# BarisYazici/deep-rl-grasping

Measured on NVIDIA H100. Metric: SAC grad-steps/sec (batch 256, 64x64 depth), higher is better.
Workload: dtype bf16x3 (fp32-faithful split, f32 accumulate)

## Files before the change

deep-rl-grasping_b200/_lib.py:

```python
from __future__ import annotations

import ctypes as C
import os

_HERE = os.path.dirname(os.path.abspath(__file__))
LIB_PATH = os.path.join(_HERE, "libb200grasp.so")

B2G_PREC_FP32_SIMT, B2G_PREC_BF16X3, B2G_PREC_BF16 = 0, 1, 2
B2G_EINVAL, B2G_ECUDA, B2G_ESTATE = -1, -2, -3

SYMBOLS = [
    "b2g_last_error", "b2g_version", "b2g_nccl_unique_id", "b2g_sac_create", "b2g_sac_destroy", "b2g_sac_dp_export", "b2g_sac_dp_connect", "b2g_debug_dp_stamps", "b2g_debug_compact_host", "b2g_sync",
    "b2g_sac_create2", "b2g_param_count", "b2g_param_info", "b2g_get_param", "b2g_set_param", "b2g_get_grad", "b2g_get_adam",
    "b2g_reset_optimizer", "b2g_replay_add", "b2g_replay_size", "b2g_replay_get", "b2g_replay_info", "b2g_get_last_batch", "b2g_set_norm_stats", "b2g_sac_step",
    "b2g_sac_step_async", "b2g_sac_step_explicit", "b2g_sac_step_host_pipelined", "b2g_sac_pipeline_flush", "b2g_sac_act", "b2g_launches_per_step", "b2g_last_step_ms",
    "b2g_profile_step", "b2g_sac_state_save", "b2g_sac_state_load",
    "b2g_sac_observe_act", "b2g_sac_observe_add", "b2g_obs_rms_set", "b2g_obs_rms_get", "b2g_upload_bytes",
    "b2g_bdq_create", "b2g_bdq_destroy", "b2g_bdq_param_count", "b2g_bdq_param_info", "b2g_bdq_get_param", "b2g_bdq_set_param",
    "b2g_bdq_get_grad", "b2g_bdq_replay_add", "b2g_bdq_replay_size", "b2g_bdq_set_norm_stats", "b2g_bdq_step",
    "b2g_bdq_step_explicit", "b2g_bdq_act", "b2g_bdq_set_per_beta", "b2g_bdq_get_last_per", "b2g_bdq_state_save", "b2g_bdq_state_load",
    "b2g_bdq_observe_act", "b2g_bdq_observe_add", "b2g_bdq_obs_rms_set", "b2g_bdq_obs_rms_get", "b2g_bdq_upload_bytes",
    "b2g_dqn_create", "b2g_dqn_destroy", "b2g_dqn_param_count", "b2g_dqn_param_info", "b2g_dqn_get_param", "b2g_dqn_set_param",
    "b2g_dqn_get_grad", "b2g_dqn_replay_add", "b2g_dqn_replay_size", "b2g_dqn_set_norm_stats", "b2g_dqn_step",
    "b2g_dqn_step_explicit", "b2g_dqn_set_per_beta", "b2g_dqn_get_last_per", "b2g_dqn_update_target", "b2g_dqn_act",
    "b2g_dqn_state_save", "b2g_dqn_state_load",
    "b2g_ppo_create", "b2g_ppo_destroy", "b2g_ppo_param_count", "b2g_ppo_param_info", "b2g_ppo_get_param", "b2g_ppo_set_param",
    "b2g_ppo_get_grad", "b2g_ppo_rollout_act", "b2g_ppo_rollout_reward", "b2g_ppo_rollout_reset", "b2g_ppo_rollout_get",
    "b2g_ppo_update", "b2g_ppo_train_step_explicit", "b2g_ppo_act", "b2g_ppo_get_step", "b2g_ppo_state_save", "b2g_ppo_state_load",
    "b2g_encoder_create", "b2g_encoder_destroy", "b2g_encoder_n_layers", "b2g_encoder_layer_shape", "b2g_encoder_set_weights",
    "b2g_encoder_encode", "b2g_debug_gemm", "b2g_debug_tensor_info", "b2g_debug_tensor",
    "b2g_autoencoder_create", "b2g_autoencoder_destroy", "b2g_autoencoder_n_layers", "b2g_autoencoder_layer_shape",
    "b2g_autoencoder_set_weights", "b2g_autoencoder_get_weights", "b2g_autoencoder_get_grad", "b2g_autoencoder_reset_optimizer",
    "b2g_autoencoder_set_dataset", "b2g_autoencoder_train_epoch", "b2g_autoencoder_evaluate", "b2g_autoencoder_predict",
    "b2g_autoencoder_step",
]

ENC_MAX_LAYERS = 8


class EncoderCfg(C.Structure):
    _fields_ = [
        ("height", C.c_int32), ("width", C.c_int32), ("channels", C.c_int32), ("n_layers", C.c_int32),
        ("filters", C.c_int32 * ENC_MAX_LAYERS), ("kernel", C.c_int32 * ENC_MAX_LAYERS), ("strides", C.c_int32 * ENC_MAX_LAYERS),
        ("encoding_dim", C.c_int32), ("alpha", C.c_float), ("max_batch", C.c_int32), ("device", C.c_int32),
    ]


class BdqCfg(C.Structure):
    _fields_ = [
        ("obs_dim", C.c_int32), ("n_branches", C.c_int32), ("n_bins", C.c_int32), ("trunk0", C.c_int32), ("trunk1", C.c_int32),
        ("branch_hidden", C.c_int32), ("batch", C.c_int32), ("buffer_capacity", C.c_int64), ("gamma", C.c_float),
        ("target_update_freq", C.c_int32), ("trunk_grad_rescale", C.c_int32), ("seed", C.c_uint64), ("device", C.c_int32),
        ("rank", C.c_int32), ("nranks", C.c_int32), ("nccl_id", C.c_void_p), ("nccl_lib", C.c_char_p),
        ("prioritized_replay", C.c_int32), ("per_alpha", C.c_float), ("per_eps", C.c_float),
    ]


class BdqMetrics(C.Structure):
    _fields_ = [("loss", C.c_float), ("mean_q", C.c_float), ("grad_norm", C.c_float), ("n_updates", C.c_int64)]

    def as_dict(self):
        return {n: getattr(self, n) for n, _ in self._fields_}


class DqnCfg(C.Structure):
    _fields_ = [
        ("obs_dim", C.c_int32), ("n_actions", C.c_int32), ("hidden0", C.c_int32), ("hidden1", C.c_int32), ("batch", C.c_int32),
        ("buffer_capacity", C.c_int64), ("gamma", C.c_float), ("seed", C.c_uint64), ("device", C.c_int32),
        ("prioritized_replay", C.c_int32), ("per_alpha", C.c_float), ("per_eps", C.c_float),
    ]


class DqnMetrics(C.Structure):
    _fields_ = [("loss", C.c_float), ("mean_q", C.c_float), ("mean_abs_td", C.c_float), ("grad_norm", C.c_float),
                ("n_clipped", C.c_int32), ("n_updates", C.c_int64)]

    def as_dict(self):
        return {n: getattr(self, n) for n, _ in self._fields_}


class PpoCfg(C.Structure):
    _fields_ = [
        ("obs_dim", C.c_int32), ("n_actions", C.c_int32), ("hidden0", C.c_int32), ("hidden1", C.c_int32), ("n_envs", C.c_int32),
        ("n_steps", C.c_int32), ("nminibatches", C.c_int32), ("noptepochs", C.c_int32), ("gamma", C.c_float), ("lam", C.c_float),
        ("ent_coef", C.c_float), ("vf_coef", C.c_float), ("max_grad_norm", C.c_float), ("seed", C.c_uint64), ("device", C.c_int32),
    ]


class PpoMetrics(C.Structure):
    _fields_ = [("policy_loss", C.c_float), ("value_loss", C.c_float), ("entropy", C.c_float), ("approxkl", C.c_float),
                ("clipfrac", C.c_float), ("grad_norm", C.c_float), ("n_updates", C.c_int64)]

    def as_dict(self):
        return {n: getattr(self, n) for n, _ in self._fields_}


class SacCfg(C.Structure):
    _fields_ = [
        ("obs_h", C.c_int32), ("obs_w", C.c_int32), ("obs_c", C.c_int32), ("obs_dim", C.c_int32),
        ("n_act", C.c_int32), ("hidden", C.c_int32), ("batch", C.c_int32), ("buffer_capacity", C.c_int64),
        ("gamma", C.c_float), ("tau", C.c_float), ("target_entropy", C.c_float), ("seed", C.c_uint64),
        ("precision", C.c_int32), ("device", C.c_int32), ("rank", C.c_int32), ("nranks", C.c_int32),
        ("nccl_id", C.c_void_p), ("nccl_lib", C.c_char_p),
    ]


class ReplayCfg(C.Structure):
    _fields_ = [("frame_capacity", C.c_int64), ("u8_plane_mask", C.c_uint32)]


class SacMetrics(C.Structure):
    _fields_ = [(n, C.c_float) for n in (
        "policy_loss", "qf1_loss", "qf2_loss", "value_loss", "ent_coef_loss", "entropy", "ent_coef",
        "grad_norm_pi", "grad_norm_values", "grad_ent", "mean_q1", "mean_q2", "mean_v", "mean_logp")] + \
        [("n_updates", C.c_int64)]

    def as_dict(self):
        return {n: getattr(self, n) for n, _ in self._fields_}


class B2GError(RuntimeError):
    def __init__(self, msg, code=None):
        super().__init__(msg)
        self.code = code


_lib = None


def load():
    global _lib
    if _lib is not None:
        return _lib
    if not os.path.exists(LIB_PATH):
        raise B2GError(f"{LIB_PATH} is missing: run ./build.sh (there is no CPU fallback for the learner path)")
    lib = C.CDLL(LIB_PATH)
    fp, dp, vp = C.POINTER(C.c_float), C.POINTER(C.c_double), C.c_void_p
    lib.b2g_last_error.restype = C.c_char_p
    lib.b2g_nccl_unique_id.argtypes = [vp, C.c_char_p]
    lib.b2g_sac_create.argtypes = [C.POINTER(SacCfg), C.POINTER(vp)]
    lib.b2g_sac_create2.argtypes = [C.POINTER(SacCfg), C.POINTER(ReplayCfg), C.POINTER(vp)]
    i64p = C.POINTER(C.c_int64)
    lib.b2g_replay_info.argtypes = [vp, i64p, i64p, i64p, i64p, i64p, i64p]
    lib.b2g_sac_destroy.argtypes = [vp]
    lib.b2g_sac_dp_export.argtypes = [vp, vp]
    lib.b2g_sac_dp_connect.argtypes = [vp, vp, C.c_int]
    lib.b2g_debug_dp_stamps.argtypes = [vp, C.POINTER(C.c_longlong)]
    lib.b2g_debug_compact_host.argtypes = [vp, vp, C.c_int, C.c_int, C.c_int, C.c_int]
    lib.b2g_sync.argtypes = [vp]
    lib.b2g_param_count.argtypes = [vp]
    lib.b2g_param_info.argtypes = [vp, C.c_int, C.POINTER(C.c_char_p), C.POINTER(C.c_int64), C.POINTER(C.c_int32),
                                   C.POINTER(C.c_int64)]
    for f in ("b2g_get_param", "b2g_set_param", "b2g_get_grad"):
        getattr(lib, f).argtypes = [vp, C.c_char_p, fp, C.c_size_t]
    lib.b2g_get_adam.argtypes = [vp, C.c_char_p, fp, fp, C.c_size_t]
    lib.b2g_reset_optimizer.argtypes = [vp]
    lib.b2g_replay_add.argtypes = [vp, fp, fp, fp, fp, fp, C.c_int64]
    lib.b2g_replay_size.argtypes = [vp]
    lib.b2g_replay_size.restype = C.c_int64
    lib.b2g_replay_get.argtypes = [vp, C.c_int64, fp, fp, fp, fp, fp]
    lib.b2g_get_last_batch.argtypes = [vp, C.POINTER(C.c_int32), fp, fp, fp]
    lib.b2g_set_norm_stats.argtypes = [vp, dp, dp, C.c_double, C.c_double, C.c_double, C.c_double, C.c_int, C.c_int]
    lib.b2g_sac_step.argtypes = [vp, C.c_int, C.c_float, C.POINTER(SacMetrics)]
    lib.b2g_sac_step_async.argtypes = [vp, C.c_int, C.c_float]
    lib.b2g_sac_step_explicit.argtypes = [vp, fp, fp, fp, fp, fp, fp, C.c_float, C.c_int, C.POINTER(SacMetrics), fp, fp]
    lib.b2g_sac_step_host_pipelined.argtypes = [vp, fp, fp, fp, fp, fp, fp, C.c_float, C.POINTER(SacMetrics), C.POINTER(C.c_int)]
    lib.b2g_sac_pipeline_flush.argtypes = [vp, C.POINTER(SacMetrics)]
    lib.b2g_sac_act.argtypes = [vp, fp, C.c_int, C.c_int, fp]
    lib.b2g_sac_observe_act.argtypes = [vp, fp, C.c_int, C.c_int, C.c_int, fp]
    lib.b2g_sac_observe_add.argtypes = [vp, fp, fp, fp, fp, fp, C.c_int, C.c_int]
    lib.b2g_obs_rms_set.argtypes = [vp, dp, dp, C.c_double]
    lib.b2g_obs_rms_get.argtypes = [vp, dp, dp, dp]
    lib.b2g_upload_bytes.argtypes = [vp, i64p, i64p]
    lib.b2g_launches_per_step.argtypes = [vp]
    lib.b2g_last_step_ms.argtypes = [vp]
    lib.b2g_last_step_ms.restype = C.c_float
    lib.b2g_profile_step.argtypes = [vp, C.c_float, C.POINTER(C.c_char_p), fp, C.c_int]
    for f in ("b2g_sac_state_save", "b2g_sac_state_load", "b2g_bdq_state_save", "b2g_bdq_state_load", "b2g_dqn_state_save",
              "b2g_dqn_state_load", "b2g_ppo_state_save", "b2g_ppo_state_load"):
        getattr(lib, f).argtypes = [vp, C.c_char_p]
    lib.b2g_bdq_create.argtypes = [C.POINTER(BdqCfg), C.POINTER(vp)]
    lib.b2g_bdq_destroy.argtypes = [vp]
    lib.b2g_bdq_param_count.argtypes = [vp]
    lib.b2g_bdq_param_info.argtypes = [vp, C.c_int, C.c_char_p, C.c_size_t, C.POINTER(C.c_int64), C.POINTER(C.c_int64), C.POINTER(C.c_int32)]
    for f in ("b2g_bdq_get_param", "b2g_bdq_set_param", "b2g_bdq_get_grad"):
        getattr(lib, f).argtypes = [vp, C.c_char_p, fp, C.c_size_t]
    lib.b2g_bdq_replay_add.argtypes = [vp, fp, fp, fp, fp, fp, C.c_int64]
    lib.b2g_bdq_replay_size.argtypes = [vp]
    lib.b2g_bdq_replay_size.restype = C.c_int64
    lib.b2g_bdq_set_norm_stats.argtypes = [vp, dp, dp, C.c_double, C.c_double, C.c_double, C.c_double, C.c_int, C.c_int]
    lib.b2g_bdq_step.argtypes = [vp, C.c_int, C.c_float, C.POINTER(BdqMetrics)]
    lib.b2g_bdq_step_explicit.argtypes = [vp, fp, fp, fp, fp, fp, fp, C.c_float, C.c_int, C.POINTER(BdqMetrics), fp]
    lib.b2g_bdq_act.argtypes = [vp, fp, C.c_int, C.POINTER(C.c_int32)]
    lib.b2g_bdq_set_per_beta.argtypes = [vp, C.c_float]
    lib.b2g_bdq_get_last_per.argtypes = [vp, C.POINTER(C.c_int32), fp, fp]
    lib.b2g_bdq_observe_act.argtypes = [vp, fp, C.c_int, C.c_int, C.c_float, C.POINTER(C.c_int32)]
    lib.b2g_bdq_observe_add.argtypes = [vp, fp, fp, fp, fp, fp, C.c_int, C.c_int]
    lib.b2g_bdq_obs_rms_set.argtypes = [vp, dp, dp, C.c_double]
    lib.b2g_bdq_obs_rms_get.argtypes = [vp, dp, dp, dp]
    lib.b2g_bdq_upload_bytes.argtypes = [vp, i64p, i64p]
    lib.b2g_dqn_create.argtypes = [C.POINTER(DqnCfg), C.POINTER(vp)]
    lib.b2g_dqn_destroy.argtypes = [vp]
    lib.b2g_dqn_param_count.argtypes = [vp]
    lib.b2g_dqn_param_info.argtypes = [vp, C.c_int, C.c_char_p, C.c_size_t, C.POINTER(C.c_int64), C.POINTER(C.c_int64), C.POINTER(C.c_int32)]
    for f in ("b2g_dqn_get_param", "b2g_dqn_set_param", "b2g_dqn_get_grad"):
        getattr(lib, f).argtypes = [vp, C.c_char_p, fp, C.c_size_t]
    lib.b2g_dqn_replay_add.argtypes = [vp, fp, fp, fp, fp, fp, C.c_int64]
    lib.b2g_dqn_replay_size.argtypes = [vp]
    lib.b2g_dqn_replay_size.restype = C.c_int64
    lib.b2g_dqn_set_norm_stats.argtypes = [vp, dp, dp, C.c_double, C.c_double, C.c_double, C.c_double, C.c_int, C.c_int]
    lib.b2g_dqn_step.argtypes = [vp, C.c_int, C.c_float, C.POINTER(DqnMetrics)]
    lib.b2g_dqn_step_explicit.argtypes = [vp, fp, fp, fp, fp, fp, fp, C.c_float, C.c_int, C.POINTER(DqnMetrics), fp]
    lib.b2g_dqn_set_per_beta.argtypes = [vp, C.c_float]
    lib.b2g_dqn_get_last_per.argtypes = [vp, C.POINTER(C.c_int32), fp, fp]
    lib.b2g_dqn_update_target.argtypes = [vp]
    lib.b2g_dqn_act.argtypes = [vp, fp, C.c_int, C.POINTER(C.c_int32), fp]
    lib.b2g_ppo_create.argtypes = [C.POINTER(PpoCfg), C.POINTER(vp)]
    lib.b2g_ppo_destroy.argtypes = [vp]
    lib.b2g_ppo_param_count.argtypes = [vp]
    lib.b2g_ppo_param_info.argtypes = [vp, C.c_int, C.c_char_p, C.c_size_t, C.POINTER(C.c_int64), C.POINTER(C.c_int64), C.POINTER(C.c_int32)]
    for f in ("b2g_ppo_get_param", "b2g_ppo_set_param", "b2g_ppo_get_grad"):
        getattr(lib, f).argtypes = [vp, C.c_char_p, fp, C.c_size_t]
    lib.b2g_ppo_rollout_act.argtypes = [vp, fp, fp]
    lib.b2g_ppo_rollout_reward.argtypes = [vp, fp, fp]
    lib.b2g_ppo_rollout_reset.argtypes = [vp]
    lib.b2g_ppo_rollout_get.argtypes = [vp, fp, fp, fp, fp, fp]
    lib.b2g_ppo_update.argtypes = [vp, fp, C.POINTER(C.c_int32), C.c_float, C.c_float, C.c_float, C.POINTER(PpoMetrics)]
    lib.b2g_ppo_train_step_explicit.argtypes = [vp, fp, fp, fp, fp, fp, C.c_float, C.c_float, C.c_float, C.c_int, C.POINTER(PpoMetrics)]
    lib.b2g_ppo_act.argtypes = [vp, fp, C.c_int, C.c_int, fp, fp, fp]
    lib.b2g_ppo_get_step.argtypes = [vp, i64p, i64p, C.POINTER(C.c_int32)]
    lib.b2g_encoder_create.argtypes = [C.POINTER(EncoderCfg), C.POINTER(vp)]
    lib.b2g_encoder_destroy.argtypes = [vp]
    lib.b2g_encoder_n_layers.argtypes = [vp]
    lib.b2g_encoder_layer_shape.argtypes = [vp, C.c_int, C.POINTER(C.c_int64), C.POINTER(C.c_int64)]
    lib.b2g_encoder_set_weights.argtypes = [vp, C.c_int, fp, C.c_size_t, fp, C.c_size_t]
    lib.b2g_encoder_encode.argtypes = [vp, fp, C.c_int, fp]
    lib.b2g_autoencoder_create.argtypes = [C.POINTER(EncoderCfg), C.POINTER(vp)]
    lib.b2g_autoencoder_destroy.argtypes = [vp]
    lib.b2g_autoencoder_n_layers.argtypes = [vp]
    lib.b2g_autoencoder_layer_shape.argtypes = [vp, C.c_int, C.POINTER(C.c_int64), C.POINTER(C.c_int64)]
    for f in ("b2g_autoencoder_set_weights", "b2g_autoencoder_get_weights", "b2g_autoencoder_get_grad"):
        getattr(lib, f).argtypes = [vp, C.c_int, fp, C.c_size_t, fp, C.c_size_t]
    lib.b2g_autoencoder_reset_optimizer.argtypes = [vp]
    lib.b2g_autoencoder_set_dataset.argtypes = [vp, fp, fp, C.c_int64]
    lib.b2g_autoencoder_train_epoch.argtypes = [vp, C.POINTER(C.c_int32), C.c_int64, C.c_int, C.c_float, dp]
    lib.b2g_autoencoder_evaluate.argtypes = [vp, C.c_int64, C.c_int64, dp]
    lib.b2g_autoencoder_predict.argtypes = [vp, fp, C.c_int, fp]
    lib.b2g_autoencoder_step.argtypes = [vp, fp, fp, C.c_int, C.c_float, C.c_int, dp]
    lib.b2g_debug_gemm.argtypes = [C.c_int, C.c_int, C.c_int, fp, fp, fp, C.c_int, C.c_int]
    lib.b2g_debug_tensor_info.argtypes = [vp, C.c_char_p, i64p, C.POINTER(C.c_int32), C.POINTER(C.c_int32)]
    lib.b2g_debug_tensor.argtypes = [vp, C.c_char_p, C.c_int, vp, C.c_size_t]
    _lib = lib
    return lib


def check(rc: int):
    if rc < 0:
        raise B2GError(f"libb200grasp error {rc}: {load().b2g_last_error().decode(errors='replace')}", rc)
    return rc


def default_nccl_lib():
    try:
        import importlib.util
        spec = importlib.util.find_spec("nvidia.nccl")
        if spec and spec.submodule_search_locations:
            p = os.path.join(list(spec.submodule_search_locations)[0], "lib", "libnccl.so.2")
            if os.path.exists(p):
                return p
    except Exception:
        pass
    return None
```

deep-rl-grasping_b200/csrc/cg.cu:

```cuda
#include <cuda_bf16.h>

#include <cstdio>
#include <cstdlib>

#include "cg.cuh"
#include "common.cuh"
#include "wgmma.cuh"

namespace b2g {
namespace {

constexpr int NMMA_WARPS = 8, NEPI_WARPS = CG_EPI_WARPS, NPROD_WARPS = 2;
constexpr int EPI_WARP0 = NMMA_WARPS, PROD_WARP0 = NMMA_WARPS + NEPI_WARPS;
static_assert(NEPI_WARPS == 4, "the epilogue is one warpgroup: one row of the 128-row tile per lane");
constexpr int NTHREADS = 32 * (PROD_WARP0 + 4);
constexpr int MMA_REGS = 168, EPI_REGS = 152, PROD_REGS = 24;
static_assert(2 * MMA_REGS + EPI_REGS + PROD_REGS <= 512, "register file");
constexpr int STG_BYTES = 2 * 64 * 16 * 4;

__device__ __forceinline__ uint32_t smem_u32(const void* p) { return (uint32_t)__cvta_generic_to_shared(p); }
__device__ __forceinline__ void mbar_init(uint32_t bar, uint32_t count) {
  asm volatile("mbarrier.init.shared::cta.b64 [%0], %1;" ::"r"(bar), "r"(count));
}
__device__ __forceinline__ void mbar_arrive(uint32_t bar) { asm volatile("mbarrier.arrive.shared::cta.b64 _, [%0];" ::"r"(bar) : "memory"); }
__device__ __forceinline__ void mbar_expect_tx(uint32_t bar, uint32_t bytes) {
  asm volatile("mbarrier.arrive.expect_tx.shared::cta.b64 _, [%0], %1;" ::"r"(bar), "r"(bytes) : "memory");
}
__device__ __forceinline__ void mbar_wait(uint32_t bar, uint32_t parity) {
  asm volatile(
      "{\n\t"
      ".reg .pred p;\n\t"
      "CG_WAIT:\n\t"
      "mbarrier.try_wait.parity.shared::cta.b64 p, [%0], %1;\n\t"
      "@p bra CG_DONE;\n\t"
      "bra CG_WAIT;\n\t"
      "CG_DONE:\n\t"
      "}" ::"r"(bar), "r"(parity)
      : "memory");
}
__device__ __forceinline__ bool elect_one() {
  uint32_t pred;
  asm volatile(
      "{\n\t"
      ".reg .pred p;\n\t"
      "elect.sync _|p, 0xffffffff;\n\t"
      "selp.u32 %0, 1, 0, p;\n\t"
      "}"
      : "=r"(pred));
  return pred != 0;
}
__device__ __forceinline__ uint64_t desc_at(uint64_t bits, uint32_t saddr) { return bits | (uint64_t)((saddr & 0x3FFFFu) >> 4); }

__device__ __forceinline__ void tma_load(uint32_t dst, const CUtensorMap* map, uint32_t bar, int rank, const int (&c)[5]) {
  switch (rank) {
    case 2:
      asm volatile("cp.async.bulk.tensor.2d.shared::cluster.global.tile.mbarrier::complete_tx::bytes [%0], [%1, {%3, %4}], [%2];" ::"r"(dst), "l"(map),
                   "r"(bar), "r"(c[0]), "r"(c[1])
                   : "memory");
      break;
    case 3:
      asm volatile("cp.async.bulk.tensor.3d.shared::cluster.global.tile.mbarrier::complete_tx::bytes [%0], [%1, {%3, %4, %5}], [%2];" ::"r"(dst),
                   "l"(map), "r"(bar), "r"(c[0]), "r"(c[1]), "r"(c[2])
                   : "memory");
      break;
    case 4:
      asm volatile("cp.async.bulk.tensor.4d.shared::cluster.global.tile.mbarrier::complete_tx::bytes [%0], [%1, {%3, %4, %5, %6}], [%2];" ::"r"(dst),
                   "l"(map), "r"(bar), "r"(c[0]), "r"(c[1]), "r"(c[2]), "r"(c[3])
                   : "memory");
      break;
    default:
      asm volatile("cp.async.bulk.tensor.5d.shared::cluster.global.tile.mbarrier::complete_tx::bytes [%0], [%1, {%3, %4, %5, %6, %7}], [%2];" ::"r"(
                       dst),
                   "l"(map), "r"(bar), "r"(c[0]), "r"(c[1]), "r"(c[2]), "r"(c[3]), "r"(c[4])
                   : "memory");
      break;
  }
}

struct CgPack { CgProblem p[CG_MAX_PROBLEMS]; };
struct Tile { int p, tm, tn, c_begin, c_end; };
struct Walker {
  int p = -1, next_start = 0, tile_start = 0, tiles_n = 1, per = 1, splits = 1, chunks = 0, cps = 0;
  __device__ __forceinline__ bool advance(const CgProblem* __restrict__ probs, int nprob, int tile) {
    bool changed = false;
    while (p < 0 || (p + 1 < nprob && tile >= next_start)) {
      ++p;
      const CgProblem& P = probs[p];
      tile_start = P.tile_start; tiles_n = P.tiles_n; per = P.tiles_m * P.tiles_n; splits = P.splits; chunks = P.chunks;
      cps = (chunks + splits - 1) / splits;
      next_start = p + 1 < nprob ? probs[p + 1].tile_start : 0x7fffffff;
      changed = true;
    }
    return changed;
  }
  __device__ __forceinline__ Tile tile(int t_abs) const {
    int t = t_abs - tile_start, split = 0;
    if (splits > 1) { split = t / per; t -= split * per; }
    Tile ti;
    ti.p = p;
    ti.tm = tiles_n == 1 ? t : t / tiles_n;
    ti.tn = t - ti.tm * tiles_n;
    ti.c_begin = split * cps;
    ti.c_end = min(chunks, ti.c_begin + cps);
    return ti;
  }
};

__device__ __forceinline__ uint32_t pack_bf16x2(float lo, float hi) {
  uint32_t d;
  asm("cvt.rn.bf16x2.f32 %0, %1, %2;" : "=r"(d) : "f"(hi), "f"(lo));
  return d;
}

template <int NT, int NPROD, int TRANS, int KS, int NACC>
__device__ __forceinline__ void mma_chunk(float (&acc)[NACC], uint32_t sbase, uint32_t a_off, uint32_t b_off, uint32_t a_ks, uint32_t b_ks,
                                          uint32_t a_ks2, uint64_t a_desc, uint64_t b_desc, uint32_t a_ps, uint32_t b_ps, uint32_t m_off) {
  constexpr int NPL = NPROD >= 6 ? 3 : (NPROD >= 3 ? 2 : 1), G = NT / 2;
  static_assert(NACC == G * NPL, "one accumulator group of NT columns per product order");
#pragma unroll
  for (int k = 0; k < KS; ++k) {
    uint64_t da[NPL], db[NPL];
#pragma unroll
    for (int pl = 0; pl < NPL; ++pl) {
      const uint32_t pa = sbase + (uint32_t)pl * a_ps + a_off + (uint32_t)(k & 1) * a_ks + (uint32_t)(k >> 1) * a_ks2 + m_off;
      const uint32_t pb = sbase + (uint32_t)pl * b_ps + b_off + (uint32_t)k * b_ks;
      da[pl] = desc_at(a_desc, pa);
      db[pl] = desc_at(b_desc, pb);
    }
    Wgmma<NT, TRANS>::mma(acc, da[0], db[0]);
    if constexpr (NPL >= 2) Wgmma<NT, TRANS>::mma(acc + G, da[0], db[1]);
    if constexpr (NPL >= 3) Wgmma<NT, TRANS>::mma(acc + 2 * G, da[0], db[2]);
    if constexpr (NPL >= 2) Wgmma<NT, TRANS>::mma(acc + G, da[1], db[0]);
    if constexpr (NPL >= 3) {
      Wgmma<NT, TRANS>::mma(acc + 2 * G, da[1], db[1]);
      Wgmma<NT, TRANS>::mma(acc + 2 * G, da[2], db[0]);
    }
  }
}

__device__ __forceinline__ void mbar_arrive_if(uint32_t bar, bool pred) {
  asm volatile(
      "{\n\t"
      ".reg .pred p;\n\t"
      "setp.ne.u32 p, %1, 0;\n\t"
      "@p mbarrier.arrive.shared::cta.b64 _, [%0];\n\t"
      "}" ::"r"(bar), "r"((uint32_t)pred)
      : "memory");
}
__device__ __forceinline__ void stamp_if(long long* dst, bool pred) {
  asm volatile(
      "{\n\t"
      ".reg .pred p;\n\t"
      ".reg .u64 t;\n\t"
      "mov.u64 t, %%clock64;\n\t"
      "setp.ne.u32 p, %1, 0;\n\t"
      "@p st.global.u64 [%0], t;\n\t"
      "}" ::"l"(dst), "r"((uint32_t)pred)
      : "memory");
}

template <int NT, int NPROD, int TRANS, int KS, class Body>
__device__ __forceinline__ void consume_tile(const CgProblem& P, const Tile& ti, uint32_t ring, uint32_t stg, int slot_bytes, int nstages, uint32_t& s,
                                             uint32_t& ph, uint64_t* bar_full, uint64_t* bar_empty, bool nomma, long long* ctrace, uint32_t& gc,
                                             bool handoff, uint32_t acc_buf, uint32_t& nb, uint64_t* acc_full, uint64_t* acc_empty, Body&& body) {
  constexpr int NGRP = NPROD >= 6 ? 3 : (NPROD >= 3 ? 2 : 1);
  constexpr int NACC = NT / 2 * NGRP;
  const int tid = threadIdx.x, lane = tid & 31, warp = tid >> 5;
  const int wg = warp >> 2, wl = warp & 3, half = wl >> 1;
  float acc[NACC];
#pragma unroll
  for (int j = 0; j < NACC; ++j) acc[j] = 0.f;
  const uint32_t a_ps = (uint32_t)P.a_pstride, b_ps = (uint32_t)P.b_pstride, a_off = P.a_off, b_off = P.b_off, a_ks = P.a_kstep, b_ks = P.b_kstep;
  const uint32_t a_ks2 = P.a_kstep2;
  const uint64_t a_desc = P.a_desc, b_desc = P.b_desc;
  const uint32_t m_off = (uint32_t)wg * (uint32_t)P.a_moff;
  uint32_t prev = 0;
  if (nomma) {
    for (int c = ti.c_begin; c < ti.c_end; ++c, ++gc) {
      mbar_wait(smem_u32(&bar_full[s]), (ph >> s) & 1u);
      mbar_arrive_if(smem_u32(&bar_empty[s]), lane == 0);
      ph ^= 1u << s;
      if (++s == (uint32_t)nstages) s = 0;
    }
  } else {
    for (int c = ti.c_begin; c < ti.c_end; ++c, ++gc) {
      long long* const tr = ctrace + gc * 8;
      const bool stamp = ctrace != nullptr && lane == 0 && gc < 64;
      stamp_if(tr + 3, stamp);
      mbar_wait(smem_u32(&bar_full[s]), (ph >> s) & 1u);
      stamp_if(tr + 4, stamp);
      wg_arrive();
      mma_chunk<NT, NPROD, TRANS, KS>(acc, ring + s * (uint32_t)slot_bytes, a_off, b_off, a_ks, b_ks, a_ks2, a_desc, b_desc, a_ps, b_ps, m_off);
      wg_commit();
      wg_wait<1>();
      mbar_arrive_if(smem_u32(&bar_empty[prev]), lane == 0 && c > ti.c_begin);
      stamp_if(tr + 5, stamp);
      prev = s;
      ph ^= 1u << s;
      if (++s == (uint32_t)nstages) s = 0;
    }
    wg_wait<0>();
    mbar_arrive_if(smem_u32(&bar_empty[prev]), lane == 0);
  }
  if constexpr (NGRP > 2) {
#pragma unroll
    for (int j = 0; j < NT / 2; ++j) acc[j] = acc[j] + (acc[j + NT / 2] + acc[j + NT]);
  } else if constexpr (NGRP > 1) {
#pragma unroll
    for (int j = 0; j < NT / 2; ++j) acc[j] = acc[j] + acc[j + NT / 2];
  }
  if (handoff) {
    mbar_wait(smem_u32(acc_empty), (nb & 1u) ^ 1u);
    const uint32_t R = 64u * wg + 16u * wl + (uint32_t)(lane >> 2), sw = (uint32_t)(lane >> 2);
    const uint32_t rowa = acc_buf + R * (uint32_t)(NT * 4) + (uint32_t)((lane & 1) * 8);
#pragma unroll
    for (int j = 0; j < NT / 8; ++j)
#pragma unroll
      for (int h = 0; h < 2; ++h) {
        const uint32_t a = rowa + (uint32_t)h * (8u * NT * 4) + ((((uint32_t)(2 * j) + (uint32_t)((lane & 3) >> 1)) ^ sw) << 4);
        asm volatile("st.shared.v2.f32 [%0], {%1,%2};" ::"r"(a), "f"(acc[4 * j + 2 * h]), "f"(acc[4 * j + 2 * h + 1]) : "memory");
      }
    __syncwarp();
    mbar_arrive_if(smem_u32(acc_full), lane == 0);
    ++nb;
    return;
  }
  const int rrow = 32 * (wl & 1) + lane;
  const uint32_t wstg = stg + (uint32_t)wg * 4096u;
#pragma unroll
  for (int R = 0; R < (NT + 63) / 64; ++R) {
    float x[32];
#pragma unroll
    for (int t = 0; t < 4; ++t) {
      const int c0 = 64 * R + 16 * t;
      if (c0 < NT) {
        asm volatile("bar.sync %0, 128;" ::"r"(1 + wg) : "memory");
#pragma unroll
        for (int jj = 0; jj < 2; ++jj)
#pragma unroll
          for (int h = 0; h < 2; ++h) {
            const int row = 16 * wl + (lane >> 2) + 8 * h, chunk = 2 * jj + ((lane & 3) >> 1);
            const int j = c0 / 8 + jj;
            const uint32_t a = wstg + (uint32_t)row * 64u + (uint32_t)((chunk ^ ((row >> 1) & 3)) << 4) + (uint32_t)((lane & 1) * 8);
            asm volatile("st.shared.v2.f32 [%0], {%1,%2};" ::"r"(a), "f"(acc[4 * j + 2 * h]), "f"(acc[4 * j + 2 * h + 1]) : "memory");
          }
        asm volatile("bar.sync %0, 128;" ::"r"(1 + wg) : "memory");
        if (half == (t >> 1)) {
#pragma unroll
          for (int cc = 0; cc < 4; ++cc) {
            const uint32_t a = wstg + (uint32_t)rrow * 64u + (uint32_t)((cc ^ ((rrow >> 1) & 3)) << 4);
            float* xd = x + 16 * (t & 1) + 4 * cc;
            asm volatile("ld.shared.v4.f32 {%0,%1,%2,%3}, [%4];" : "=f"(xd[0]), "=f"(xd[1]), "=f"(xd[2]), "=f"(xd[3]) : "r"(a));
          }
        }
      }
    }
    const int g = 2 * R + half;
    if (32 * g < NT) body(g, x);
  }
}

struct RowOff {
  long long roff = 0, rmoff = 0;
  int ri0 = 0, ri1 = 0;
  bool ok = true;
  __device__ __forceinline__ void set(const CgProblem& Q, int r) {
    const int d0 = Q.d0, d1 = Q.d1;
    const int i0 = r % d0, i12 = r / d0, i1 = i12 % d1, i2 = i12 / d1;
    roff = Q.o_base + (long long)i0 * Q.o0 + (long long)i1 * Q.o1 + (long long)i2 * Q.o2;
    if (Q.rgrp_rows > 0) roff += Q.rgrp_off[min(r / Q.rgrp_rows, 7)];
    rmoff = Q.m_base + (long long)i0 * Q.m0 + (long long)i1 * Q.m1 + (long long)i2 * Q.m2;
    ri0 = i0; ri1 = i1;
    ok = Q.lim_i0 <= 0 || i0 < Q.lim_i0;
  }
};

__global__ void __launch_bounds__(NTHREADS, 1)
cg_kernel(const __grid_constant__ CgPack pk, int nprob, int total_tiles, const CUtensorMap* __restrict__ maps, int max_stages,
          int dbg, long long* __restrict__ trace) {
  const CgProblem* __restrict__ probs = pk.p;
  extern __shared__ uint8_t smem_raw[];
  __shared__ __align__(8) uint64_t bar_full[CG_MAX_STAGES], bar_empty[CG_MAX_STAGES], acc_full, acc_empty;
  const int tid = threadIdx.x, lane = tid & 31;
  const int warp = __shfl_sync(0xffffffffu, tid >> 5, 0);
  const int trace_cta = dbg >> 8;
  const bool dbg_noload = dbg & 1, dbg_nomma = dbg & 2, dbg_nostore = dbg & 4, dbg_nost = dbg & 16;
  if (tid == 0) {
    for (int s = 0; s < max_stages; ++s) { mbar_init(smem_u32(&bar_full[s]), 1); mbar_init(smem_u32(&bar_empty[s]), NMMA_WARPS); }
    mbar_init(smem_u32(&acc_full), NMMA_WARPS);
    mbar_init(smem_u32(&acc_empty), NEPI_WARPS);
    asm volatile("fence.mbarrier_init.release.cluster;" ::: "memory");
  }
  __syncthreads();
  const uint32_t stg = (smem_u32(smem_raw) + 1023u) & ~1023u;
  const uint32_t ring = stg + STG_BYTES;
  pdl_trigger();
  pdl_wait();

  if (warp >= PROD_WARP0) {
    asm volatile("setmaxnreg.dec.sync.aligned.u32 %0;" ::"n"(PROD_REGS));
    const int pw = warp - PROD_WARP0;
    if (pw >= NPROD_WARPS) return;
    {
      uint32_t gc = 0, s = 0, ph = 0, nbuf = 0;
      int slot_bytes = 0, nstages = 1;
      bool handoff = false;
      Walker w;
      int n2 = 1, nloads = 0, planes = 0, tx = 0;
      const int* tab = nullptr;
      for (int tile = blockIdx.x; tile < total_tiles; tile += gridDim.x) {
        if (w.advance(probs, nprob, tile)) {
          const CgProblem& P = probs[w.p];
          n2 = P.n2; nloads = P.nloads; planes = P.planes; tx = P.tx_bytes; tab = P.tm_tab; handoff = cg_epi_handoff(P.epi);
          if (P.slot_bytes != slot_bytes || P.nstages != nstages) {
            for (int q = 0; q < nstages; ++q) mbar_wait(smem_u32(&bar_empty[q]), ((ph >> q) & 1u) ^ 1u);
            if (nbuf) {
              mbar_wait(smem_u32(&acc_full), (nbuf - 1) & 1u);
              mbar_wait(smem_u32(&acc_empty), (nbuf - 1) & 1u);
              asm volatile("fence.proxy.async.shared::cta;" ::: "memory");
            }
            slot_bytes = P.slot_bytes; nstages = P.nstages; s = 0;
          }
        }
        const Tile ti = w.tile(tile);
        const CgProblem& P = probs[ti.p];
        if (handoff && ti.c_end > ti.c_begin) ++nbuf;
        if (P.dep_ctr) {
          const int* __restrict__ ctr = P.dep_ctr;
          const int x0 = P.dep_by_chunk ? ti.c_begin : ti.tm, x1 = P.dep_by_chunk ? ti.c_end : ti.tm + 1;
          const int lo = x0 * P.dep_rows / P.dep_rows_tile, hi = min(P.dep_tiles - 1, (x1 * P.dep_rows - 1) / P.dep_rows_tile);
          const int expect = P.dep_expect * NEPI_WARPS;
          for (int j = lo + lane; j <= hi; j += 32) {
            int seen;
            do {
              asm volatile("ld.acquire.gpu.global.s32 %0, [%1];" : "=r"(seen) : "l"(ctr + j) : "memory");
              if (seen < expect) __nanosleep(100);
            } while (seen < expect);
          }
          __syncwarp();
          asm volatile("fence.proxy.async.global;" ::: "memory");
        }
        int base[CG_MAX_LOADS][5];
#pragma unroll
        for (int l = 0; l < CG_MAX_LOADS; ++l) {
          if (l < nloads) {
            const CgLoad& L = P.ld[l];
#pragma unroll
            for (int d = 0; d < 5; ++d) base[l][d] = L.c0[d] + ti.tm * L.d_tm[d] + ti.tn * L.d_tn[d];
            if (tab) { base[l][1] += tab[(ti.tm * CG_MAX_LOADS + l) * 2]; base[l][2] += tab[(ti.tm * CG_MAX_LOADS + l) * 2 + 1]; }
          }
        }
        int c1 = n2 > 1 ? ti.c_begin / n2 : 0, c2 = ti.c_begin - c1 * n2;
        for (int c = ti.c_begin; c < ti.c_end; ++c, ++gc) {
          const bool tr = trace && blockIdx.x == trace_cta && pw == 0 && gc < 64 && lane == 0;
          if (tr) trace[gc * 8 + 0] = clock64();
          mbar_wait(smem_u32(&bar_empty[s]), ((ph >> s) & 1u) ^ 1u);
          if (tr) trace[gc * 8 + 1] = clock64();
          const uint32_t full = smem_u32(&bar_full[s]);
          const bool leader = elect_one();
          if (dbg_noload) { if (pw == 0 && leader) mbar_arrive(full); }
          else {
            if (pw == 0 && leader) mbar_expect_tx(full, (uint32_t)tx);
            const uint32_t sbase = ring + s * (uint32_t)slot_bytes;
            int j = 0;
#pragma unroll
            for (int l = 0; l < CG_MAX_LOADS; ++l) {
              if (l < nloads) {
                const CgLoad& L = P.ld[l];
                int crd[5];
#pragma unroll
                for (int d = 0; d < 5; ++d) crd[d] = base[l][d] + c1 * L.d_c1[d] + c2 * L.d_c2[d];
                if (L.plane_box) {
                  if ((j & (NPROD_WARPS - 1)) == pw && leader) tma_load(sbase + (uint32_t)L.smem_off, maps + L.map, full, L.rank, crd);
                  ++j;
                } else {
                  for (int pl = 0; pl < planes; ++pl, ++j) {
#pragma unroll
                    for (int d = 2; d < 5; ++d) if (d == L.rank - 1) crd[d] = pl;
                    if ((j & (NPROD_WARPS - 1)) == pw && leader)
                      tma_load(sbase + (uint32_t)(pl * L.plane_stride + L.smem_off), maps + L.map, full, L.rank, crd);
                  }
                }
              }
            }
          }
          if (tr) { trace[gc * 8 + 2] = clock64(); trace[gc * 8 + 6] = ti.p * 100000 + ti.tm * 10 + ti.tn; }
          if (++c2 == n2) { c2 = 0; ++c1; }
          ph ^= 1u << s;
          if (++s == (uint32_t)nstages) s = 0;
        }
      }
    }
  } else if (warp < NMMA_WARPS) {
    asm volatile("setmaxnreg.inc.sync.aligned.u32 %0;" ::"n"(MMA_REGS));
    const int q = 2 * (warp >> 2) + (warp & 1);
    uint32_t it = 0, s = 0, ph = 0, gc = 0, nb = 0;
    int slot_bytes = 0, nstages = 1;
    Walker w;
    long long* const ctrace = trace && blockIdx.x == trace_cta && warp == 0 ? trace : nullptr;
    const int r = q * 32 + lane;
    int epi = 0, rows_tile = 0, lim_rows = 0, umma_n = 0, n_valid = 0, shape = 0;
    bool handoff = false;
    uint32_t acc_buf = 0;
    long long o_tm = 0;
    RowOff ro;
    for (int tile = blockIdx.x; tile < total_tiles; tile += gridDim.x) {
      if (w.advance(probs, nprob, tile)) {
        const CgProblem& Q = probs[w.p];
        epi = Q.epi; rows_tile = Q.rows_tile; lim_rows = Q.lim_rows; umma_n = Q.umma_n; n_valid = Q.n_valid; o_tm = Q.o_tm;
        ro.set(Q, r);
        shape = cg_shape_key(Q.umma_n, Q.nprod, Q.mn_major != 0, Q.ksteps);
        if (Q.slot_bytes != slot_bytes || Q.nstages != nstages) { slot_bytes = Q.slot_bytes; nstages = Q.nstages; s = 0; }
        handoff = cg_epi_handoff(epi);
        acc_buf = ring + (uint32_t)(nstages * slot_bytes);
      }
      const Tile ti = w.tile(tile);
      if (ti.c_end <= ti.c_begin) continue;
      const CgProblem& P = probs[ti.p];
      const bool valid0 = r < rows_tile && ti.tm * rows_tile + r < lim_rows && ro.ok;
      const long long off0 = ro.roff + (long long)ti.tm * o_tm;
      const int n0 = ti.tn * umma_n;
      const bool tre = trace && blockIdx.x == trace_cta && warp == 0 && lane == 0 && it < 16;
      if (tre) trace[512 + it * 4 + 0] = clock64();
      auto body = [&](int g, float (&x)[32]) {
        const int ng = n0 + 32 * g;
        if (dbg_nostore || ng >= n_valid || !valid0) return;
        float* dst = P.out_f + off0 + (long long)(ng >> 5) * P.f_grp;
        if (epi == CG_EPI_RAW) {
          if (P.atomic) {
#pragma unroll
            for (int j = 0; j < 8; ++j)
              asm volatile("red.global.add.v4.f32 [%0], {%1,%2,%3,%4};" ::"l"(dst + 4 * j), "f"(x[4 * j]), "f"(x[4 * j + 1]), "f"(x[4 * j + 2]),
                           "f"(x[4 * j + 3])
                           : "memory");
          } else {
#pragma unroll
            for (int j = 0; j < 8; ++j) *reinterpret_cast<float4*>(dst + 4 * j) = make_float4(x[4 * j], x[4 * j + 1], x[4 * j + 2], x[4 * j + 3]);
          }
          return;
        }
        const float sc = P.scale;
        if (P.atomic) {
#pragma unroll
          for (int j = 0; j < 8; ++j)
            asm volatile("red.global.add.v4.f32 [%0], {%1,%2,%3,%4};" ::"l"(dst + 4 * j), "f"(x[4 * j] * sc), "f"(x[4 * j + 1] * sc),
                         "f"(x[4 * j + 2] * sc), "f"(x[4 * j + 3] * sc)
                         : "memory");
        } else {
#pragma unroll
          for (int j = 0; j < 8; ++j)
            *reinterpret_cast<float4*>(dst + 4 * j) = make_float4(x[4 * j] * sc, x[4 * j + 1] * sc, x[4 * j + 2] * sc, x[4 * j + 3] * sc);
          if (P.dp_n > 1) {
            const int i4 = (int)((dst - P.dp_gbase) >> 2), per4 = P.dp_per4;
#pragma unroll
            for (int j = 0; j < 8; ++j) {
              const int owner = (i4 + j) / per4;
              if (owner != P.dp_rank)
                reinterpret_cast<float4*>(P.dp_recv[owner])[(size_t)P.dp_rank * per4 + (i4 + j - owner * per4)] =
                    make_float4(x[4 * j] * sc, x[4 * j + 1] * sc, x[4 * j + 2] * sc, x[4 * j + 3] * sc);
            }
          }
        }
      };
#define CG_CONSUME(NT, NPROD, TRANS, KS)                                                                                                      \
  consume_tile<NT, NPROD, TRANS, KS>(P, ti, ring, stg, slot_bytes, nstages, s, ph, bar_full, bar_empty, dbg_nomma, ctrace, gc, handoff, acc_buf, \
                                     nb, &acc_full, &acc_empty, body)
      switch (shape) {
        case cg_shape_key(32, 6, false, 4): CG_CONSUME(32, 6, 0, 4); break;
        case cg_shape_key(64, 6, false, 4): CG_CONSUME(64, 6, 0, 4); break;
        case cg_shape_key(64, 3, false, 4): CG_CONSUME(64, 3, 0, 4); break;
        case cg_shape_key(128, 3, false, 4): CG_CONSUME(128, 3, 0, 4); break;
        case cg_shape_key(64, 3, true, 4): CG_CONSUME(64, 3, 1, 4); break;
        case cg_shape_key(64, 3, true, 9): CG_CONSUME(64, 3, 1, 9); break;
        case cg_shape_key(128, 3, true, 4): CG_CONSUME(128, 3, 1, 4); break;
        default: __trap();
      }
#undef CG_CONSUME
      if (tre) {
        trace[512 + it * 4 + 1] = clock64();
        trace[512 + it * 4 + 2] = handoff;
        trace[512 + it * 4 + 3] = ti.p * 100000 + ti.tm * 10 + ti.tn;
      }
      ++it;
    }
  } else {
    asm volatile("setmaxnreg.inc.sync.aligned.u32 %0;" ::"n"(EPI_REGS));
    const int ew = warp - EPI_WARP0;
    const int r = ew * 32 + lane;
    uint32_t ne = 0;
    int slot_bytes = 0, nstages = 1;
    Walker w;
    int epi = 0, rows_tile = 0, lim_rows = 0, umma_n = 0, out_planes = 0, grp_stride = 32, n_valid = 0, grp_tab = 0;
    bool handoff = false;
    uint32_t acc_buf = 0;
    long long o_tm = 0, m_tm = 0;
    RowOff ro;
    const float* __restrict__ bias = nullptr;
    const uint16_t* __restrict__ mask = nullptr;
    for (int tile = blockIdx.x; tile < total_tiles; tile += gridDim.x) {
      if (w.advance(probs, nprob, tile)) {
        const CgProblem& Q = probs[w.p];
        epi = Q.epi; rows_tile = Q.rows_tile; lim_rows = Q.lim_rows; umma_n = Q.umma_n; out_planes = Q.out_planes;
        grp_stride = Q.grp_stride; n_valid = Q.n_valid; o_tm = Q.o_tm; m_tm = Q.m_tm; bias = Q.bias; mask = Q.mask; grp_tab = Q.grp_tab;
        ro.set(Q, r);
        if (Q.slot_bytes != slot_bytes || Q.nstages != nstages) { slot_bytes = Q.slot_bytes; nstages = Q.nstages; }
        handoff = cg_epi_handoff(epi);
        acc_buf = ring + (uint32_t)(nstages * slot_bytes);
      }
      const Tile ti = w.tile(tile);
      if (ti.c_end <= ti.c_begin || !handoff) continue;
      const CgProblem& P = probs[ti.p];
      bool valid0 = r < rows_tile && ti.tm * rows_tile + r < lim_rows && ro.ok;
      long long off0 = ro.roff + (long long)ti.tm * o_tm;
      const long long moff0 = ro.rmoff + (long long)ti.tm * m_tm;
      if (P.tm_sub > 1) {
        const int tq = ti.tm / P.tm_sub, tr = ti.tm - tq * P.tm_sub;
        off0 = ro.roff + (long long)tq * o_tm + (long long)tr * P.o_sub;
        valid0 = valid0 && tr * P.d1 + ro.ri1 < P.lim_i1;
      }
      const int n0 = ti.tn * umma_n, ngroups = umma_n >> 5;
      auto group_at = [&](int g, bool& valid, long long& off, long long& moff) {
        const int ng = n0 + 32 * g;
        valid = valid0; off = off0; moff = moff0;
        if (grp_tab) {
          const int gg = ng >> 5;
          valid = valid0 && ro.ri0 < P.grp_lim0[gg] && ro.ri1 < P.grp_lim1[gg];
          off = off0 + P.grp_off[gg]; moff = moff0 + P.grp_moff[gg] - ng;
        }
      };
      const bool tre = trace && blockIdx.x == trace_cta && ew == 0 && lane == 0 && ne < 16;
      if (tre) trace[576 + ne * 4 + 0] = clock64();
      uint32_t mbits[4] = {0u, 0u, 0u, 0u};
      if (epi == CG_EPI_DGRAD && !dbg_nostore) {
#pragma unroll
        for (int g = 0; g < 4; ++g) {
          bool valid;
          long long off, moff;
          group_at(g, valid, off, moff);
          const int ng = n0 + 32 * g;
          if (g < ngroups && valid && ng < n_valid) {
            uint4 mk[4];
#pragma unroll
            for (int j = 0; j < 4; ++j) mk[j] = __ldg(reinterpret_cast<const uint4*>(mask + moff + ng) + j);
#pragma unroll
            for (int j = 0; j < 4; ++j) {
              const uint32_t wd[4] = {mk[j].x, mk[j].y, mk[j].z, mk[j].w};
#pragma unroll
              for (int uu = 0; uu < 4; ++uu) {
                if (wd[uu] & 0x00007FFFu) mbits[g] |= 1u << (8 * j + 2 * uu);
                if (wd[uu] & 0x7FFF0000u) mbits[g] |= 1u << (8 * j + 2 * uu + 1);
              }
            }
          }
        }
      }
      mbar_wait(smem_u32(&acc_full), ne & 1u);
      if (tre) trace[576 + ne * 4 + 1] = clock64();
      const bool split_fin = P.ws != nullptr;
      float* __restrict__ wsrow = split_fin ? P.ws + ((size_t)(ti.tm * w.tiles_n + ti.tn) * 128 + r) * umma_n : nullptr;
      auto body = [&](int g, float (&x)[32], int pass) {
        const int ng = n0 + 32 * g;
        bool valid;
        long long off, moff;
        group_at(g, valid, off, moff);
        if (pass == 0 && split_fin) {
#pragma unroll
          for (int j = 0; j < 8; ++j)
            asm volatile("red.global.add.v4.f32 [%0], {%1,%2,%3,%4};" ::"l"(wsrow + 32 * g + 4 * j), "f"(x[4 * j]), "f"(x[4 * j + 1]), "f"(x[4 * j + 2]),
                         "f"(x[4 * j + 3])
                         : "memory");
          return;
        }
        const bool live = !dbg_nostore && ng < n_valid;
        float4 bv[8];
        if (epi == CG_EPI_ACT && live) {
#pragma unroll
          for (int j = 0; j < 8; ++j) bv[j] = __ldg(reinterpret_cast<const float4*>(bias + (long long)(ng >> 5) * P.bias_grp) + j);
        }
        if (!live) return;
        if (epi == CG_EPI_ACT) {
#pragma unroll
          for (int j = 0; j < 8; ++j) {
            x[4 * j] = fmaxf(x[4 * j] + bv[j].x, 0.f); x[4 * j + 1] = fmaxf(x[4 * j + 1] + bv[j].y, 0.f);
            x[4 * j + 2] = fmaxf(x[4 * j + 2] + bv[j].z, 0.f); x[4 * j + 3] = fmaxf(x[4 * j + 3] + bv[j].w, 0.f);
          }
          if (P.f0 > 0 && valid && !dbg_nost) {
            float* dst = P.out_f + (long long)ti.tm * P.f_tm + (long long)r * P.f0 + (long long)(ng >> 5) * P.f_grp;
#pragma unroll
            for (int j = 0; j < 8; ++j) *reinterpret_cast<float4*>(dst + 4 * j) = make_float4(x[4 * j], x[4 * j + 1], x[4 * j + 2], x[4 * j + 3]);
          }
        } else {
          const uint32_t mb = g == 0 ? mbits[0] : g == 1 ? mbits[1] : g == 2 ? mbits[2] : mbits[3];
#pragma unroll
          for (int j = 0; j < 32; ++j)
            if (!((mb >> j) & 1u)) x[j] = 0.f;
          if (P.colsum) {
            float cs[32];
#pragma unroll
            for (int j = 0; j < 32; ++j) cs[j] = x[j];
#pragma unroll
            for (int wd = 16; wd >= 1; wd >>= 1) {
              const bool up = (lane & wd) != 0;
#pragma unroll
              for (int j = 0; j < wd; ++j) {
                const float send = up ? cs[j] : cs[j + wd], keep = up ? cs[j + wd] : cs[j];
                cs[j] = keep + __shfl_xor_sync(0xffffffffu, send, wd);
              }
            }
            atomicAdd(P.colsum + ((ng + lane) & P.colsum_mask), cs[0]);
          }
        }
        const long long gcol = grp_tab ? 0 : (long long)(ng >> 5) * grp_stride;
        const long long roff = off + gcol;
        const int q0 = lane & ~3, qi = lane & 3;
#pragma unroll 1
        for (int pl = 0; pl < out_planes; ++pl) {
          uint32_t pk[16];
#pragma unroll
          for (int j = 0; j < 16; ++j) {
            pk[j] = pack_bf16x2(x[2 * j], x[2 * j + 1]);
            x[2 * j] -= __uint_as_float(pk[j] << 16);
            x[2 * j + 1] -= __uint_as_float(pk[j] & 0xFFFF0000u);
          }
          if (dbg_nost) continue;
#pragma unroll
          for (int m = 1; m <= 2; m <<= 1) {
            const bool up = (lane & m) != 0;
#pragma unroll
            for (int c0 = 0; c0 < 4; ++c0) {
              if (c0 & m) continue;
              const int c1 = c0 | m;
#pragma unroll
              for (int u = 0; u < 4; ++u) {
                const uint32_t got = __shfl_xor_sync(0xffffffffu, up ? pk[4 * c0 + u] : pk[4 * c1 + u], m);
                if (up) pk[4 * c0 + u] = got; else pk[4 * c1 + u] = got;
              }
            }
          }
          uint16_t* const base = P.out_p[pl];
#pragma unroll
          for (int j = 0; j < 4; ++j) {
            const long long oj = __shfl_sync(0xffffffffu, roff, q0 + j);
            const bool vj = __shfl_sync(0xffffffffu, valid ? 1 : 0, q0 + j) != 0;
            if (vj) *reinterpret_cast<uint4*>(base + oj + 8 * qi) = make_uint4(pk[4 * j], pk[4 * j + 1], pk[4 * j + 2], pk[4 * j + 3]);
          }
        }
      };
      const uint32_t rowa = acc_buf + (uint32_t)(r * umma_n * 4), sw = (uint32_t)(r & 7);
      for (int g = 0; g < ngroups; ++g) {
        float x[32];
#pragma unroll
        for (int cc = 0; cc < 8; ++cc) {
          const uint32_t a = rowa + ((((uint32_t)(8 * g + cc)) ^ sw) << 4);
          asm volatile("ld.shared.v4.f32 {%0,%1,%2,%3}, [%4];" : "=f"(x[4 * cc]), "=f"(x[4 * cc + 1]), "=f"(x[4 * cc + 2]), "=f"(x[4 * cc + 3]) : "r"(a));
        }
        if (g == ngroups - 1) {
          __syncwarp();
          mbar_arrive_if(smem_u32(&acc_empty), lane == 0);
        }
        body(g, x, 0);
      }
      ++ne;
      bool last_arriver = !split_fin;
      if (split_fin) {
        __syncwarp();
        int old = 0;
        if (lane == 0) { __threadfence(); old = atomicAdd(P.ws_cnt + (ti.tm * w.tiles_n + ti.tn) * NEPI_WARPS + ew, 1); }
        old = __shfl_sync(0xffffffffu, old, 0);
        last_arriver = old == w.splits - 1;
        if (last_arriver) {
          __threadfence();
          if (lane == 0) P.ws_cnt[(ti.tm * w.tiles_n + ti.tn) * NEPI_WARPS + ew] = 0;
          for (int g = 0; g < ngroups; ++g) {
            float x[32];
#pragma unroll
            for (int j = 0; j < 8; ++j) {
              const float4 sum = __ldcg(reinterpret_cast<const float4*>(wsrow + 32 * g) + j);
              x[4 * j] = sum.x; x[4 * j + 1] = sum.y; x[4 * j + 2] = sum.z; x[4 * j + 3] = sum.w;
              __stcg(reinterpret_cast<float4*>(wsrow + 32 * g) + j, make_float4(0.f, 0.f, 0.f, 0.f));
            }
            body(g, x, 1);
          }
        }
      }
      __syncwarp();
      if (lane == 0 && P.done_ctr && last_arriver) {
        __threadfence();
        atomicAdd(P.done_ctr + ti.tm, 1);
      }
      if (tre) { trace[576 + (ne - 1) * 4 + 2] = clock64(); trace[576 + (ne - 1) * 4 + 3] = ti.p * 100000 + ti.tm * 10 + ti.tn; }
    }
  }
}

typedef CUresult (*EncodeTiledFn)(CUtensorMap*, CUtensorMapDataType, cuuint32_t, void*, const cuuint64_t*, const cuuint64_t*, const cuuint32_t*,
                                  const cuuint32_t*, CUtensorMapInterleave, CUtensorMapSwizzle, CUtensorMapL2promotion, CUtensorMapFloatOOBfill);
EncodeTiledFn g_encode = nullptr;

}

bool cg_shape_supported(int umma_n, int nprod, bool mn_major, int ksteps) {
  switch (cg_shape_key(umma_n, nprod, mn_major, ksteps)) {
    case cg_shape_key(32, 6, false, 4): case cg_shape_key(64, 6, false, 4): case cg_shape_key(64, 3, false, 4): case cg_shape_key(128, 3, false, 4):
    case cg_shape_key(64, 3, true, 4): case cg_shape_key(64, 3, true, 9): case cg_shape_key(128, 3, true, 4): return true;
    default: return false;
  }
}

int cg_smem_limit() { return 226 * 1024 - STG_BYTES; }

int cg_encode_map(CUtensorMap* out, const void* base, int rank, const uint64_t* dims, const uint64_t* strides_bytes, const uint32_t* box,
                  const uint32_t* elem_strides, int swizzle) {
  if (swizzle != 128 && swizzle != 64) return -1;
  if (!g_encode) {
    cudaDriverEntryPointQueryResult q;
    void* fn = nullptr;
    if (cudaGetDriverEntryPoint("cuTensorMapEncodeTiled", &fn, cudaEnableDefault, &q) != cudaSuccess || !fn || q != cudaDriverEntryPointSuccess) return -1;
    g_encode = (EncodeTiledFn)fn;
  }
  cuuint64_t gd[5], gs[5];
  cuuint32_t bx[5], es[5];
  for (int i = 0; i < rank; ++i) { gd[i] = dims[i]; bx[i] = box[i]; es[i] = elem_strides ? elem_strides[i] : 1; }
  for (int i = 0; i + 1 < rank; ++i) gs[i] = strides_bytes[i];
  const CUresult r = g_encode(out, CU_TENSOR_MAP_DATA_TYPE_BFLOAT16, (cuuint32_t)rank, const_cast<void*>(base), gd, gs, bx, es, CU_TENSOR_MAP_INTERLEAVE_NONE,
                              swizzle == 128 ? CU_TENSOR_MAP_SWIZZLE_128B : CU_TENSOR_MAP_SWIZZLE_64B, CU_TENSOR_MAP_L2_PROMOTION_L2_256B,
                              CU_TENSOR_MAP_FLOAT_OOB_FILL_NONE);
  return r == CUDA_SUCCESS ? 0 : (int)r;
}

unsigned long long cg_desc_bits(int swizzle, bool mn_major, int lbo) {
  const unsigned long long l = mn_major ? (unsigned)lbo : 16u, sbo = 8u * (unsigned)swizzle;
  return ((l >> 4) & 0x3FFF) << 16 | ((sbo >> 4) & 0x3FFF) << 32 | (unsigned long long)(swizzle == 128 ? 1 : 2) << 62;
}

int cg_finalize(CgGroup& g, int smem_budget) {
  int start = 0, slot = 0;
  g.flops = 0;
  for (int i = 0; i < g.n; ++i) {
    CgProblem& P = g.host[i];
    P.tile_start = start;
    start += P.tiles_m * P.tiles_n * P.splits;
    for (int l = 0; l < P.nloads; ++l) {
      CgLoad& L = P.ld[l];
      L.plane_stride = L.smem_off >= P.b_off ? P.b_pstride : P.a_pstride;
      if (L.plane_box && L.box_bytes != L.plane_stride) return -2;
    }
    const int need = P.b_off + P.planes * P.b_pstride;
    P.slot_bytes = (need + 1023) / 1024 * 1024;
    slot = slot > P.slot_bytes ? slot : P.slot_bytes;
  }
  g.total_tiles = start;
  const int avail = smem_budget - 1024 ;
  g.slot_bytes = slot; g.nstages = 0;
  int ring = 0;
  for (int i = 0; i < g.n; ++i) {
    CgProblem& P = g.host[i];
    const int acc = cg_epi_handoff(P.epi) ? cg_acc_bytes(P.umma_n) : 0;
    const int avail_ring = avail - acc;
    P.nstages = P.slot_bytes > 0 ? avail_ring / P.slot_bytes : 0;
    if (P.nstages > CG_MAX_STAGES) P.nstages = CG_MAX_STAGES;
    if (P.nstages < 2) return -1;
    P.slot_bytes = avail_ring / P.nstages / 1024 * 1024;
    g.nstages = g.nstages > P.nstages ? g.nstages : P.nstages;
    ring = ring > P.nstages * P.slot_bytes + acc ? ring : P.nstages * P.slot_bytes + acc;
  }
  g.ring_bytes = ring;
  return 0;
}

long long* g_cg_trace = nullptr;

cudaError_t cg_launch(const CgGroup& g, const CUtensorMap* dev_maps, int num_sms, cudaStream_t s, bool pdl, int debug_flags) {
  if (g.total_tiles <= 0 || (debug_flags & 8)) return cudaSuccess;
  static bool attr_set = false;
  if (!attr_set) {
    cudaError_t e = cudaFuncSetAttribute(cg_kernel, cudaFuncAttributeMaxDynamicSharedMemorySize, 226 * 1024);
    if (e != cudaSuccess) return e;
    attr_set = true;
  }
  const int smem = 1024 + STG_BYTES + g.ring_bytes;
  const int grid = g.total_tiles < num_sms ? g.total_tiles : num_sms;
  CgPack pk;
  static_assert(sizeof(CgPack) < 28 * 1024, "problem list must fit the kernel parameter space (32,764 B)");
  for (int i = 0; i < g.n; ++i) pk.p[i] = g.host[i];
  cudaError_t e = launch_pdl(cg_kernel, dim3(grid), dim3(NTHREADS), (size_t)smem, s, pdl, pk, g.n, g.total_tiles, dev_maps, g.nstages, debug_flags, g_cg_trace);
  if (e != cudaSuccess) fprintf(stderr, "cg_launch %s: %s (grid %d, %d threads, smem %d)\n", g.name, cudaGetErrorString(e), grid, NTHREADS, smem);
  return e;
}

}
```

deep-rl-grasping_b200/csrc/cg.cuh:

```cuda
#pragma once
#include <cuda.h>
#include <cuda_runtime.h>
#include <stdint.h>

namespace b2g {

constexpr int CG_MAX_LOADS = 4;
constexpr int CG_MAX_PROBLEMS = 16;
constexpr int CG_MAX_STAGES = 8;
constexpr int CG_MAX_PLANES = 3;
constexpr int CG_EPI_WARPS = 4;

enum CgEpiKind : int {
  CG_EPI_ACT = 0,
  CG_EPI_RAW = 1,
  CG_EPI_DGRAD = 2,
  CG_EPI_WGRAD = 3,
};
__host__ __device__ constexpr bool cg_epi_handoff(int epi) { return epi == CG_EPI_ACT || epi == CG_EPI_DGRAD; }
__host__ __device__ constexpr int cg_acc_bytes(int umma_n) { return 128 * umma_n * 4; }

struct CgLoad {
  int map;
  int rank;
  int box_bytes;
  int smem_off;
  int plane_stride;
  int plane_box;
  int c0[5];
  int d_tm[5], d_tn[5], d_c1[5], d_c2[5];
};

struct CgProblem {
  int tile_start, tiles_m, tiles_n, splits;
  int chunks, n2;
  int nloads, planes;
  int a_pstride, b_pstride;
  int tx_bytes;
  int slot_bytes, nstages;
  CgLoad ld[CG_MAX_LOADS];
  const int* tm_tab;
  int mn_major;
  unsigned long long a_desc, b_desc;
  int a_moff;
  int ksteps;
  int a_off, b_off;
  int a_kstep, b_kstep;
  int a_kstep2;
  int a_lbo, b_lbo;
  int umma_n;
  int nprod;
  int epi;
  int rows_tile;
  int lim_rows;
  int d0, d1;
  long long o_tm; int o0, o1, o2; long long o_base;
  int rgrp_rows;
  int rgrp_off[8];
  int lim_i0;
  int tm_sub;
  long long o_sub;
  int lim_i1;
  long long m_tm; int m0, m1, m2; long long m_base;
  int n_valid;
  int grp_stride;
  int grp_tab;
  int grp_off[8], grp_moff[8], grp_lim0[8], grp_lim1[8];
  int out_planes;
  uint16_t* out_p[CG_MAX_PLANES];
  float* out_f;
  long long f_tm; int f0;
  const float* bias;
  int bias_grp;
  long long f_grp;
  const uint16_t* mask;
  float* colsum;
  int colsum_mask;
  int atomic;
  float scale;
  int* done_ctr;
  const int* dep_ctr;
  int dep_rows, dep_rows_tile, dep_tiles, dep_expect;
  float* ws;
  int* ws_cnt;
  float* dp_recv[8];
  const float* dp_gbase;
  int dp_rank, dp_n, dp_per4;
  int dep_by_chunk;
};

struct CgGroup {
  CgProblem host[CG_MAX_PROBLEMS];
  int n = 0;
  int total_tiles = 0;
  int slot_bytes = 0, nstages = 0, ring_bytes = 0;
  const char* name = "";
  double flops = 0;
};

int cg_encode_map(CUtensorMap* out, const void* base, int rank, const uint64_t* dims, const uint64_t* strides_bytes, const uint32_t* box,
                  const uint32_t* elem_strides, int swizzle = 128);
unsigned long long cg_desc_bits(int swizzle, bool mn_major, int lbo);
int cg_finalize(CgGroup& g, int smem_budget);
cudaError_t cg_launch(const CgGroup& g, const CUtensorMap* dev_maps, int num_sms, cudaStream_t s, bool pdl, int debug_flags);
int cg_smem_limit();
__host__ __device__ constexpr int cg_shape_key(int umma_n, int nprod, bool mn_major, int ksteps) {
  return ksteps * 8192 + umma_n * 16 + nprod * 2 + (mn_major ? 1 : 0);
}
bool cg_shape_supported(int umma_n, int nprod, bool mn_major, int ksteps);

}
```

deep-rl-grasping_b200/csrc/engine_v2.cu:

```cuda
#include <cuda_bf16.h>

#include <algorithm>
#include <cstdio>
#include <cstdlib>
#include <cstring>

#include "sac_internal.cuh"

namespace b2g {
namespace {

struct Gather2Args {
  GatherArgs g;
  uint16_t* s1[2][3];
  uint16_t* fp[3][3];
  int KF;
};

__device__ __forceinline__ void split3(float y, uint16_t& p0, uint16_t& p1, uint16_t& p2) {
  const __nv_bfloat16 h0 = __float2bfloat16_rn(y);
  const float r1 = y - __bfloat162float(h0);
  const __nv_bfloat16 h1 = __float2bfloat16_rn(r1);
  const float r2 = r1 - __bfloat162float(h1);
  p0 = __bfloat16_as_ushort(h0); p1 = __bfloat16_as_ushort(h1); p2 = __bfloat16_as_ushort(__float2bfloat16_rn(r2));
}

template <int Ci>
__device__ __forceinline__ void s2d_half_block(const Gather2Args& a, const unsigned char* __restrict__ src, int it, int which, size_t b) {
  constexpr int CP = s2d_channels(Ci);
  const GatherArgs& g = a.g;
  const int npx = g.H * g.W * Ci;
  const int h = it & 1, X = (it >> 1) & 15, Y = it >> 5;
  const double clip_obs = g.normc[1];
  const bool norm_obs = g.normc[3] != 0.0;
  const float scale = g.scale;
#pragma unroll
  for (int rr = 0; rr < 2; ++rr) {
    const int e0 = ((4 * Y + 2 * h + rr) * g.W + 4 * X) * Ci;
    float y[4 * Ci];
#pragma unroll
    for (int q = 0; q < Ci; ++q) {
      const int e = e0 + 4 * q;
      const float4 v = frame_load4(src, g.fmt, npx, Ci, e);
      float t[4] = {v.x, v.y, v.z, v.w};
      if (norm_obs) {
        const double2 m0 = *reinterpret_cast<const double2*>(g.mean + e), m1 = *reinterpret_cast<const double2*>(g.mean + e + 2);
        const double2 i0 = *reinterpret_cast<const double2*>(g.var + e), i1 = *reinterpret_cast<const double2*>(g.var + e + 2);
        t[0] = (float)fmin(fmax(((double)t[0] - m0.x) * i0.x, -clip_obs), clip_obs);
        t[1] = (float)fmin(fmax(((double)t[1] - m0.y) * i0.y, -clip_obs), clip_obs);
        t[2] = (float)fmin(fmax(((double)t[2] - m1.x) * i1.x, -clip_obs), clip_obs);
        t[3] = (float)fmin(fmax(((double)t[3] - m1.y) * i1.y, -clip_obs), clip_obs);
      }
#pragma unroll
      for (int j = 0; j < 4; ++j) y[4 * q + j] = t[j];
    }
    uint32_t p[3][2 * CP];
#pragma unroll
    for (int k = 0; k < 4 * CP; k += 2) {
      uint16_t q[3][2];
#pragma unroll
      for (int u = 0; u < 2; ++u) {
        const int c = (k + u) / CP, ci = (k + u) % CP;
        if (ci < Ci) split3(y[c * Ci + ci] / scale, q[0][u], q[1][u], q[2][u]);
        else q[0][u] = q[1][u] = q[2][u] = 0;
      }
#pragma unroll
      for (int pl = 0; pl < 3; ++pl) p[pl][k / 2] = (uint32_t)q[pl][0] | ((uint32_t)q[pl][1] << 16);
    }
    const size_t o = b * 4096 * CP + (size_t)((Y * 16 + X) * 16 + 4 * (2 * h + rr)) * CP;
#pragma unroll
    for (int pl = 0; pl < 3; ++pl) {
      if constexpr (CP == 1) {
        *reinterpret_cast<uint2*>(a.s1[which][pl] + o) = make_uint2(p[pl][0], p[pl][1]);
      } else {
        uint4* d = reinterpret_cast<uint4*>(a.s1[which][pl] + o);
        d[0] = make_uint4(p[pl][0], p[pl][1], p[pl][2], p[pl][3]);
        d[1] = make_uint4(p[pl][4], p[pl][5], p[pl][6], p[pl][7]);
      }
    }
  }
}

template <int Ci>
__global__ void __launch_bounds__(512) gather2_kernel(Gather2Args a) {
  const GatherArgs& g = a.g;
  const int b = blockIdx.x, which = blockIdx.y, tid = threadIdx.x;
  const int HW = g.H * g.W, npx = HW * Ci;
  const int Ec = npx + 4;
  long long slot = b;
  if (g.indices) slot = g.indices[b];
  else if (g.rng_counters) {
    slot = philox_slot(g.seed, (unsigned long long)g.rng_counters[4], b, (unsigned long long)g.rng_counters[5]);
    if (g.ring_cap > 0) slot = ring_slot(g.rng_counters[6], (int)slot, g.ring_cap);
    if (g.indices_out && which == 0 && tid == 0) g.indices_out[b] = (int)slot;
  }
  const unsigned char* __restrict__ src =
      g.obs_frame ? g.frames + (size_t)(which ? g.next_frame : g.obs_frame)[slot] * g.frame_bytes
                  : reinterpret_cast<const unsigned char*>((which ? g.next_obs : g.obs) + (size_t)slot * Ec);
  const double clip_obs = g.normc[1];
  const bool norm_obs = g.normc[3] != 0.0;
  const float scale = g.scale;
  for (int it = tid; it < 512; it += blockDim.x) s2d_half_block<Ci>(a, src, it, which, b);
  if (tid == 0) {
    float yy = frame_elem(src, g.fmt, npx, Ci, npx);
    if (norm_obs) yy = (float)fmin(fmax(((double)yy - g.mean[npx]) * g.var[npx], -clip_obs), clip_obs);
    yy = yy / scale;
    uint16_t p0, p1, p2;
    split3(yy, p0, p1, p2);
    const size_t fo = (size_t)b * g.FS + g.feat_col, po = (size_t)b * a.KF + g.feat_col;
    if (which) { g.F_t[fo] = yy; a.fp[2][0][po] = p0; a.fp[2][1][po] = p1; a.fp[2][2][po] = p2; }
    else {
      g.F_pi[fo] = yy; g.F_v[fo] = yy;
      a.fp[0][0][po] = p0; a.fp[0][1][po] = p1; a.fp[0][2][po] = p2;
      a.fp[1][0][po] = p0; a.fp[1][1][po] = p1; a.fp[1][2][po] = p2;
    }
  }
  if (which == 0 && g.act) {
    const int feat_dim = g.feat_col + 1;
    if (tid < g.n_act) {
      const float av = g.act[slot * g.n_act + tid];
      g.F_v[(size_t)b * g.FS + feat_dim + tid] = av;
      uint16_t p0, p1, p2;
      split3(av, p0, p1, p2);
      const size_t po = (size_t)b * a.KF + feat_dim + tid;
      a.fp[1][0][po] = p0; a.fp[1][1][po] = p1; a.fp[1][2][po] = p2;
    }
    if (tid == 32) {
      float r = g.rew[slot];
      if (g.normc[4] != 0.0) r = (float)fmin(fmax((double)r * g.normc[0], -g.normc[2]), g.normc[2]);
      g.rew_out[b] = r;
      g.done_out[b] = g.done[slot];
    }
  }
}

struct Plane2Job {
  const float* src;
  uint16_t* dst[3];
  int R, N, np;
  int transpose;
  int ld, off0;
  int k1_ci;
  int tile_start;
};

constexpr int P2_SUB = 4;
__global__ void __launch_bounds__(256) planes2_kernel(const Plane2Job* __restrict__ jobs, const int* __restrict__ cta_job, int cta0) {
  __shared__ float tile[P2_SUB][64][33];
  const int cta = cta0 + blockIdx.x;
  const Plane2Job job = jobs[cta_job[cta]];
  const int t = cta - job.tile_start;
  const int strips_n = (job.N + 32 * P2_SUB - 1) / (32 * P2_SUB);
  const int r0 = (t / strips_n) * 64, nb = (t % strips_n) * 32 * P2_SUB;
  const int tid = threadIdx.x;
  const bool vec_ok = (job.N & 3) == 0;
  float4 v[P2_SUB][2];
#pragma unroll
  for (int q = 0; q < P2_SUB; ++q)
#pragma unroll
// ... 535 lines not shown
        CgProblem P = mnmajor(NB, 64, 2, 1, (B + 3) / 4);
        P.nloads = 3;
        for (int a = 0; a < 2; ++a) { P.ld[a] = mk_load(mA, 4, a * P.a_lbo); P.ld[a].d_c2[3] = 4; }
        P.ld[2] = mk_load(mB, 2, P.b_off); P.ld[2].d_c2[1] = 64;
        P.tm_tab = dtab;
        P.tiles_m = 5; P.tiles_n = 1;
        P.splits = std::max(1, std::min(P.chunks, std::max(14, (P.chunks + 15) / 16)));
        P.lim_rows = 576; P.o_tm = 128 * 64; P.o0 = 64; P.n_valid = 64;
        P.out_f = h->g(std::string(nets[n]) + "/cnn3/w"); P.atomic = 1;
        g.host[g.n++] = P;
      }
    }
    if (int rc = push_group(h, v.bwd_groups, g, "conv3_bwd")) return rc;
  }
  {
    CgGroup g;
    for (int n = 0; n < 2; ++n) {
      const int mA = add_maps(v, v.dZ2[n], NB, 4, {64, 6, 6, (uint64_t)B}, {128, 768, 4608}, {64, 8, 8, 2});
      const int mB = add_maps(v, v.W2n[n], NB, 2, {64, 512}, {128}, {64, 64}, {}, false);
      if (mA < 0 || mB < 0) return b2g_fail(B2G_ECUDA, "engine v2: cuTensorMapEncodeTiled failed (conv2 dgrad)");
      CgProblem P = kmajor(NB, 128, 4, 2, 128);
      P.tx_bytes = NB * (128 * 128 + 2 * 64 * 128);
      P.nloads = 3;
      P.ld[0] = mk_load(mA, 4, 0); P.ld[0].d_tm[3] = 2; P.ld[0].d_c1[2] = -1; P.ld[0].d_c2[1] = -1;
      for (int py = 0; py < 2; ++py) {
        P.ld[1 + py] = mk_load(mB, 2, P.b_off + py * 64 * 128);
        P.ld[1 + py].c0[1] = py * 128; P.ld[1 + py].d_c1[1] = 256; P.ld[1 + py].d_c2[1] = 64;
      }
      P.tiles_m = (B + 1) / 2;
      P.epi = CG_EPI_DGRAD; P.rows_tile = 128; P.lim_rows = B * 64;
      P.d0 = 8; P.d1 = 8;
      P.o_tm = 2 * 225 * 64; P.o0 = 2 * 64; P.o1 = 2 * 15 * 64; P.o2 = 225 * 64; P.o_base = n * 32;
      P.m_tm = 2 * 225 * 32; P.m0 = 2 * 32; P.m1 = 2 * 15 * 32; P.m2 = 225 * 32; P.m_base = 0;
      P.grp_tab = 1;
      for (int py = 0; py < 2; ++py)
        for (int px = 0; px < 2; ++px) {
          const int gg = py * 2 + px;
          P.grp_off[gg] = (py * 15 + px) * 64; P.grp_moff[gg] = (py * 15 + px) * 32;
          P.grp_lim0[gg] = (15 - px + 1) / 2; P.grp_lim1[gg] = (15 - py + 1) / 2;
        }
      P.n_valid = 128; P.out_planes = 2;
      for (int p = 0; p < 2; ++p) P.out_p[p] = v.dZ1[p];
      P.mask = v.H1[n][0];
      P.colsum = h->g(std::string(nets[n]) + "/cnn1/b"); P.colsum_mask = 31;
      g.host[g.n++] = P;
    }
    if (int rc = push_group(h, v.bwd_groups, g, "conv2_dgrad")) return rc;
  }
  {
    CgGroup g;
    for (int n = 0; n < 2; ++n) {
      const int mA = add_maps(v, v.H1[n], NB, 4, {64, 14, 15, (uint64_t)B}, {64, 15 * 64, 225 * 64}, {64, 12, 12, 4}, {1, 2, 2, 1});
      const int mB = add_maps(v, v.dZ2[n], NB, 2, {64, (uint64_t)B * 36}, {128}, {64, 144});
      if (mA < 0 || mB < 0) return b2g_fail(B2G_ECUDA, "engine v2: cuTensorMapEncodeTiled failed (conv2 wgrad)");
      CgProblem P = mnmajor(NB, 144, 2, 1, (B + 3) / 4);
      P.nloads = 3;
      for (int a = 0; a < 2; ++a) { P.ld[a] = mk_load(mA, 4, a * P.a_lbo); P.ld[a].c0[1] = 2 * a; P.ld[a].d_tm[2] = 1; P.ld[a].d_c2[3] = 4; }
      P.ld[2] = mk_load(mB, 2, P.b_off); P.ld[2].d_c2[1] = 144;
      P.tiles_m = 4; P.tiles_n = 1;
      P.splits = std::max(1, std::min(P.chunks, std::max(8, (P.chunks + 7) / 8)));
      P.lim_rows = 512; P.o_tm = 128 * 64; P.o0 = 64; P.n_valid = 64;
      P.out_f = h->g(std::string(nets[n]) + "/cnn2/w"); P.atomic = 1;
      g.host[g.n++] = P;
    }
    {
      const int mA = Cp == 1 ? add_maps(v, v.S[0], NB, 3, {32, 15, (uint64_t)B * 16}, {32, 512}, {32, 16, 4}, {}, true, 64)
                             : add_maps(v, v.S[0], NB, 3, {64, 16, (uint64_t)B * 16}, {128, 2048}, {64, 16, 4});
      const int mB = add_maps(v, v.dZ1, NB, 4, {64, 15, 15, (uint64_t)B}, {128, 15 * 128, 225 * 128}, {64, 16, 4, 1});
      if (mA < 0 || mB < 0) return b2g_fail(B2G_ECUDA, "engine v2: cuTensorMapEncodeTiled failed (conv1 wgrad)");
      CgProblem P = mnmajor(NB, 64, 2, 1, 4 * B);
      P.n2 = 4;
      if (Cp == 1) {
        P.a_pstride = 64 * 64; P.a_lbo = NB * P.a_pstride;
        P.b_off = 2 * P.a_lbo;
        P.tx_bytes = NB * (2 * 64 * 64 + 64 * 128);
        P.a_kstep = 16 * 64; P.a_kstep2 = 2 * P.a_kstep; P.a_desc = cg_desc_bits(64, true, P.a_lbo); P.a_moff = 0;
        P.nloads = 3;
        for (int a = 0; a < 2; ++a) { P.ld[a] = mk_load(mA, 3, a * P.a_lbo); P.ld[a].c0[2] = a; P.ld[a].d_c1[2] = 16; P.ld[a].d_c2[2] = 4; }
        P.tiles_m = 1;
        P.d0 = 4; P.d1 = 4; P.o0 = 32; P.o1 = 8 * 32;
        P.rgrp_rows = 16;
        for (int l = 0; l < 4; ++l) P.rgrp_off[l] = (32 * (l >> 1) + 4 * (l & 1)) * 32;
      } else {
        for (int l = 0; l < 2; ++l) {
          P.ld[l] = mk_load(mA, 3, l * P.a_lbo); P.ld[l].c0[1] = l; P.ld[l].d_tm[2] = 1; P.ld[l].d_c1[2] = 16; P.ld[l].d_c2[2] = 4;
        }
        P.nloads = 3;
        P.tiles_m = 2;
        P.d0 = 4; P.d1 = 4; P.o0 = 32; P.o1 = Ci * 32; P.o_tm = 32 * Ci * 32;
        P.lim_i0 = Ci;
        P.rgrp_rows = 16;
        for (int j = 0; j < 8; ++j) P.rgrp_off[j] = (8 * Ci * (j & 3) + 4 * Ci * (j >> 2)) * 32;
      }
      P.ld[P.nloads - 1] = mk_load(mB, 4, P.b_off); P.ld[P.nloads - 1].d_c1[3] = 1; P.ld[P.nloads - 1].d_c2[2] = 4;
      P.tiles_n = 1;
      P.splits = std::max(1, std::min(P.chunks, std::max(84 / P.tiles_m, (P.chunks + 15) / 16)));
      P.lim_rows = 64 * Cp; P.n_valid = 64;
      P.out_f = h->g("model/pi/cnn1/w"); P.f_grp = (long long)(h->g("model/values_fn/cnn1/w") - h->g("model/pi/cnn1/w")); P.atomic = 1;
      g.host[g.n++] = P;
    }
    if (int rc = push_group(h, v.bwd_groups, g, "conv_wgrad")) return rc;
  }
  int n_ctr = 0;
  {
    std::vector<const CgGroup*> parts;
    for (auto& g : v.fwd) parts.push_back(&g);
    std::vector<Wire> w;
    for (int n = 0; n < 3; ++n) {
      w.push_back({1, n, 0, n < 2 ? 0 : 1, 6, 1, 0});
      w.push_back({2, n, 1, n, 8 * 36, 108, 0});
      w.push_back({3, n, 2, n, 128 * 16, 128, 0});
      w.push_back({4, n, 3, n, 128, 128, 0});
    }
    if (int rc = fuse_groups(h, parts, w, "fwd_fused", v.fwd_fused, n_ctr)) return rc;
  }
  {
    std::vector<const CgGroup*> parts;
    for (auto& g : v.bwd_groups) parts.push_back(&g);
    std::vector<Wire> w;
    for (int n = 0; n < 2; ++n) {
      w.push_back({1, 2 * n, 0, n, 128, 128, 0});
      w.push_back({1, 2 * n + 1, 0, n, 64, 128, 1});
      w.push_back({2, 2 * n, 1, 2 * n, 3, 128, 0});
      w.push_back({2, 2 * n + 1, 1, 2 * n, 4, 128, 1});
      w.push_back({3, n, 2, 2 * n, 72, 108, 0});
      w.push_back({4, n, 2, 2 * n, 144, 108, 1});
    }
    w.push_back({4, 2, 3, 0, 1, 8, 1});
    w.push_back({4, 2, 3, 1, 1, 8, 1});
    if (int rc = fuse_groups(h, parts, w, "bwd_fused", v.bwd_fused, n_ctr)) return rc;
    std::vector<const CgGroup*> pa(parts.begin(), parts.begin() + 2), pb(parts.begin() + 2, parts.end());
    std::vector<Wire> wa, wb;
    for (int n = 0; n < 2; ++n) {
      wa.push_back({1, 2 * n, 0, n, 128, 128, 0});
      wa.push_back({1, 2 * n + 1, 0, n, 64, 128, 1});
      wb.push_back({1, n, 0, 2 * n, 72, 108, 0});
      wb.push_back({2, n, 0, 2 * n, 144, 108, 1});
    }
    wb.push_back({2, 2, 1, 0, 1, 8, 1});
    wb.push_back({2, 2, 1, 1, 1, 8, 1});
    if (int rc = fuse_groups(h, pa, wa, "bwd_fused_fc", v.bwd_fused, n_ctr)) return rc;
    if (int rc = fuse_groups(h, pb, wb, "bwd_fused_conv", v.bwd_fused, n_ctr)) return rc;
  }
  if (int rc = dev_alloc(h->allocs, h->stream, &v.dep_ctr, (size_t)n_ctr)) return rc;
  v.n_dep_ctr = n_ctr;
  bind_counters(v.fwd_fused, v.dep_ctr);
  bind_counters(v.bwd_fused, v.dep_ctr);
  if (int rc = dev_alloc(h->allocs, h->stream, &v.d_maps, v.maps.size())) return rc;
  CK(cudaMemcpyAsync(v.d_maps, v.maps.data(), v.maps.size() * sizeof(CUtensorMap), cudaMemcpyHostToDevice, h->stream));
  CK(cudaStreamSynchronize(h->stream));
  return 0;
}

int v2_planes(b2g_sac* h, bool backward, cudaStream_t s) {
  V2State& v = h->v2;
  const int cta0 = backward ? v.plane_ctas_fwd : 0, n = backward ? v.plane_ctas - v.plane_ctas_fwd : v.plane_ctas_fwd;
  planes2_kernel<<<n, 256, 0, s>>>((const Plane2Job*)v.plane_jobs, v.plane_cta_job, cta0);
  return 0;
}

int v2_gather(b2g_sac* h, const GatherArgs& ga, cudaStream_t s) {
  V2State& v = h->v2;
  Gather2Args a{};
  a.g = ga;
  for (int w = 0; w < 2; ++w)
    for (int p = 0; p < 3; ++p) a.s1[w][p] = v.S[w][p];
  for (int n = 0; n < 3; ++n) for (int p = 0; p < 3; ++p) a.fp[n][p] = v.F[n][p];
  a.KF = v.KF;
  const dim3 grid(ga.B, ga.next_obs || ga.next_frame ? 2 : 1);
  switch (h->Cimg) {
    case 1: gather2_kernel<1><<<grid, 512, 0, s>>>(a); break;
    case 2: gather2_kernel<2><<<grid, 512, 0, s>>>(a); break;
    case 3: gather2_kernel<3><<<grid, 512, 0, s>>>(a); break;
    default: gather2_kernel<4><<<grid, 512, 0, s>>>(a); break;
  }
  return 0;
}

extern long long* g_cg_trace;
static long long* s_trace_buf = nullptr;

int v2_launch(b2g_sac* h, const CgGroup& g, cudaStream_t s) {
  const char* tn = getenv("B2G_CG_TRACE");
  cudaStreamCaptureStatus cs0 = cudaStreamCaptureStatusNone;
  if (tn) cudaStreamIsCapturing(s, &cs0);
  if (tn && cs0 == cudaStreamCaptureStatusNone && std::string(tn) == g.name) {
    if (!s_trace_buf) cudaMalloc(&s_trace_buf, 640 * sizeof(long long));
    cudaMemsetAsync(s_trace_buf, 0, 640 * sizeof(long long), s);
    g_cg_trace = s_trace_buf;
    const char* tc = getenv("B2G_CG_TRACE_CTA");
    cudaError_t e = cg_launch(g, h->v2.d_maps, h->num_sms - h->v2.sm_reserve, s, false, h->v2.dbg | ((tc ? atoi(tc) : 0) << 8));
    g_cg_trace = nullptr;
    if (e != cudaSuccess) return b2g_fail(B2G_ECUDA, cudaGetErrorString(e));
    static int shots = 0;
    if (shots++ == 3) {
      long long t[640];
      cudaStreamSynchronize(s);
      cudaMemcpy(t, s_trace_buf, sizeof(t), cudaMemcpyDeviceToHost);
      const long long t0 = t[0];
      fprintf(stderr, "cg trace %s (cycles; per chunk: prod wait_start wait_done issued | mma wait_start full_seen committed)\n", g.name);
      for (int i = 0; i < 64 && t[i * 8 + 2]; ++i)
        fprintf(stderr, "  chunk %2d (p %lld tm %lld): %7lld %7lld %7lld | %7lld %7lld %7lld\n", i, t[i * 8 + 6] / 100000, t[i * 8 + 6] % 100000 / 10, t[i * 8] - t0,
                t[i * 8 + 1] - t0, t[i * 8 + 2] - t0, t[i * 8 + 3] - t0, t[i * 8 + 4] - t0, t[i * 8 + 5] - t0);
      for (int i = 0; i < 16 && t[512 + i * 4 + 1]; ++i)
        fprintf(stderr, "  tile %d (p %lld tm %lld) mma: start %7lld sums out %7lld (%s)\n", i, t[512 + i * 4 + 3] / 100000, t[512 + i * 4 + 3] % 100000 / 10,
                t[512 + i * 4] - t0, t[512 + i * 4 + 1] - t0, t[512 + i * 4 + 2] ? "handed off" : "in place");
      for (int i = 0; i < 16 && t[576 + i * 4 + 2]; ++i)
        fprintf(stderr, "  handoff %d (p %lld tm %lld) epilogue warpgroup: buffer wait %7lld start %7lld end %7lld\n", i, t[576 + i * 4 + 3] / 100000,
                t[576 + i * 4 + 3] % 100000 / 10, t[576 + i * 4] - t0, t[576 + i * 4 + 1] - t0, t[576 + i * 4 + 2] - t0);
    }
    return 0;
  }
  CK(cg_launch(g, h->v2.d_maps, h->num_sms - h->v2.sm_reserve, s, pdl_enabled(), h->v2.dbg));
  return 0;
}

}
```

deep-rl-grasping_b200/csrc/sac.cu:

```cuda
#include <cuda_runtime.h>
#include <math.h>
#include <stdio.h>
#include <string.h>

#include <algorithm>
#include <chrono>
#include <map>
#include <tuple>
#include <string>
#include <vector>

#include "../../include/b200grasp.h"
#include "common.cuh"
#include "sac_internal.cuh"
#include "state.cuh"

using namespace b2g;

namespace b2g {
bool pdl_enabled() {
  static int v = -1;
  if (v < 0) { const char* e = getenv("B2G_PDL"); v = (e && e[0] == '0') ? 0 : 1; }
  return v != 0;
}
// ... 1119 lines not shown
    h->Ec = h->Hi * h->Wi * h->Cimg + 4;
    h->feat_dim = 513;
  } else {
    if (cfg->obs_dim < 1) { delete h; return b2g_fail(B2G_EINVAL, "obs_dim must be positive for the MLP policy"); }
    h->E = h->Ec = cfg->obs_dim;
    h->feat_dim = cfg->obs_dim;
  }
  h->FS = (h->feat_dim + h->A + 7) / 8 * 8;
  auto bail = [&](int rc) { std::string keep = g_b2g_err; b2g_sac_destroy(h); g_b2g_err = keep; return rc; };
  if (cudaStreamCreateWithFlags(&h->stream, cudaStreamNonBlocking) != cudaSuccess) return bail(b2g_fail(B2G_ECUDA, "cudaStreamCreate failed"));
  cudaEventCreate(&h->ev0); cudaEventCreate(&h->ev1);
  build_params(h);
  int rc = 0;
  const int B = h->B;
#define DA(ptr, count) if ((rc = dev_alloc(h->allocs, h->stream, &(ptr), (size_t)(count)))) return bail(rc)
  DA(h->P, h->n_all); DA(h->Mo, h->n_train); DA(h->Vo, h->n_train); DA(h->G, h->n_train + MET_COUNT);
  DA(h->metrics, MET_COUNT); DA(h->counters, 8); DA(h->step_consts, 4); DA(h->d_lr, 1);
  const int64_t cap = cfg->buffer_capacity;
  {
    h->v2.on = h->cnn && cfg->precision == B2G_PREC_BF16X3 && h->Hi == 64 && h->Wi == 64 && h->Cimg <= 4;
    if (const char* dbg = getenv("B2G_CG_DEBUG")) h->v2.dbg = atoi(dbg);
  }
  {
    const int npx = h->cnn ? h->Hi * h->Wi * h->Cimg : 0, HW = h->Hi * h->Wi;
    h->row_fmt.n32 = h->Cimg; h->row_fmt.tail = 4 * npx;
    h->u8_mask = replay ? replay->u8_plane_mask : 0;
    h->fmt = h->row_fmt;
    h->frame_bytes = (int64_t)h->Ec * 4;
    if (h->u8_mask) {
      FrameFmt& f = h->fmt;
      f.n8 = f.n32 = 0;
      for (int c = 0; c < h->Cimg; ++c) f.ch[c] = (h->u8_mask >> c & 1) ? (signed char)f.n8++ : (signed char)(-1 - f.n32++);
      f.f32_off = HW * f.n8;
      f.tail = f.f32_off + 4 * HW * f.n32;
      if (f.f32_off % 16 != 0) return bail(b2g_fail(B2G_EINVAL, "8-bit planes need H * W * (8-bit planes) to be a multiple of 16"));
      h->frame_bytes = (f.tail + 16 + 15) / 16 * 16;
    }
    h->frame_cap = replay ? replay->frame_capacity : 2 * cap;
    if (h->frame_cap > INT32_MAX) return bail(b2g_fail(B2G_EINVAL, "frame_capacity must fit in int32 (frame indices)"));
    h->dedup = h->frame_cap < 2 * cap;
  }
  if ((rc = dev_alloc(h->allocs, h->stream, &h->frames, (size_t)(h->frame_cap * h->frame_bytes)))) return bail(rc);
  DA(h->r_ofr, cap); DA(h->r_nfr, cap); DA(h->r_act, cap * h->A); DA(h->r_rew, cap); DA(h->r_done, cap);
  h->stage_rows = std::max(B, 256);
  if (h->cnn) DA(h->obs_stage, (size_t)h->stage_rows * h->E);
  DA(h->c_obs, (size_t)h->stage_rows * h->Ec); DA(h->c_next, (size_t)h->stage_rows * h->Ec); DA(h->d_plan, 4 * h->stage_rows);
  if (cudaMallocHost((void**)&h->h_plan, 4 * h->stage_rows * sizeof(int)) != cudaSuccess ||
      cudaMallocHost((void**)&h->h_rc, 2 * sizeof(long long)) != cudaSuccess)
    return bail(b2g_fail(B2G_ECUDA, "replay staging"));
  DA(h->d_mean, h->Ec); DA(h->d_istd, h->Ec); DA(h->d_normc, 8);
  for (int k = 0; k < 2; ++k) {
    if (cudaMallocHost((void**)&h->hp_stats[k], (size_t)(2 * h->Ec + 8) * sizeof(double)) != cudaSuccess ||
        cudaEventCreateWithFlags(&h->ev_stats[k], cudaEventDisableTiming) != cudaSuccess)
      return bail(b2g_fail(B2G_ECUDA, "norm-stat staging"));
  }
  DA(h->s_obs, (size_t)B * h->Ec); DA(h->s_next, (size_t)B * h->Ec); DA(h->s_act, B * h->A); DA(h->s_rew, B); DA(h->s_done, B);
  if (h->cnn) {
    DA(h->x_obs, (size_t)B * h->Hi * h->Wi * h->Cimg); DA(h->x_next, (size_t)B * h->Hi * h->Wi * h->Cimg);
    for (int n = 0; n < 3; ++n) {
      DA(h->h1[n], (size_t)B * h->H1 * h->W1 * 32); DA(h->h2[n], (size_t)B * h->H2 * h->W2 * 64); DA(h->h3[n], (size_t)B * 1024);
    }
    for (int n = 0; n < 2 && !h->v2.on; ++n) {
      DA(h->dZ4[n], (size_t)B * 512); DA(h->dZ3p[n], (size_t)B * (h->H3 + 4) * (h->W3 + 4) * 64);
      DA(h->dZ2p[n], (size_t)B * (h->H2 + 3) * (h->W2 + 3) * 64); DA(h->dZ1[n], (size_t)B * h->H1 * h->W1 * 32);
    }
  }
  h->use_planes = h->cnn && cfg->precision != B2G_PREC_FP32_SIMT;
  if (h->v2.on && (rc = v2_alloc(h))) return bail(rc);
  if (h->use_planes) {
    const size_t nx = (size_t)B * h->Hi * h->Wi * h->Cimg;
    for (int k = 0; k < 2; ++k) { DA(h->xp[0][k], nx); DA(h->xp[1][k], nx); }
    for (int n = 0; n < 3; ++n)
      for (int k = 0; k < 2; ++k) {
        if (h->v2.on) {
          h->h1p[n][k] = h->v2.H1[n][k]; h->h2p[n][k] = h->v2.H2[n][k]; h->h3p[n][k] = h->v2.H3[n][k];
          continue;
        }
        DA(h->h1p[n][k], (size_t)B * h->H1 * h->W1 * 32); DA(h->h2p[n][k], (size_t)B * h->H2 * h->W2 * 64); DA(h->h3p[n][k], (size_t)B * 1024);
      }
    for (int n = 0; n < 2 && !h->v2.on; ++n)
      for (int k = 0; k < 2; ++k) {
        DA(h->dZ4p[n][k], (size_t)B * 512); DA(h->dZ3pp[n][k], (size_t)B * (h->H3 + 4) * (h->W3 + 4) * 64);
        DA(h->dZ2pp[n][k], (size_t)B * (h->H2 + 3) * (h->W2 + 3) * 64);
        DA(h->dZ1p[n][k], (size_t)B * h->H1 * h->W1 * 32);
      }
    const size_t wsz[4] = {(size_t)64 * h->Cimg * 32, 512 * 64, 576 * 64, 1024 * 512};
    for (int n = 0; n < 3; ++n)
      for (int l = 0; l < 4; ++l)
        for (int k = 0; k < 4; ++k) {
          if (n == 2 && k < 2) continue;
          DA(h->wp[n][l][k], wsz[l]);
        }
  }
  for (int n = 0; n < 3; ++n) DA(h->F[n], (size_t)B * h->FS);
  DA(h->z0[0], 5 * B * h->H);
  for (int q = 1; q < 5; ++q) h->z0[q] = h->z0[0] + (size_t)q * B * h->H;
  for (int q = 0; q < 4; ++q) { DA(h->a0[q], B * h->H); DA(h->dz1[q], B * h->H); }
  DA(h->dz0_pi, B * h->H); DA(h->dz0_v3, B * 3 * h->H);
  DA(h->per_sample, 7 * B); DA(h->pi_out, B * h->A); DA(h->eps, B * h->A + 4); DA(h->rew_n, B); DA(h->done_n, B);
  DA(h->indices, B + 4);
#undef DA
  if (cudaMallocHost((void**)&h->h_met, (MET_COUNT + 2) * sizeof(float)) != cudaSuccess ||
      cudaMallocHost((void**)&h->h_cnt, 8 * sizeof(long long)) != cudaSuccess)
    return bail(b2g_fail(B2G_ECUDA, "cudaMallocHost failed"));
  for (int j = 0; j < 2; ++j) {
    if ((rc = dev_alloc(h->allocs, h->stream, &h->ps_obs[j], (size_t)B * h->Ec)) || (rc = dev_alloc(h->allocs, h->stream, &h->ps_next[j], (size_t)B * h->Ec))) return bail(rc);
    if (cudaEventCreateWithFlags(&h->ev_h2d[j], cudaEventDisableTiming) != cudaSuccess ||
        cudaEventCreateWithFlags(&h->ev_consumed[j], cudaEventDisableTiming) != cudaSuccess ||
        cudaEventCreateWithFlags(&h->ev_met[j], cudaEventDisableTiming) != cudaSuccess ||
        cudaMallocHost((void**)&h->pm_met[j], (MET_COUNT + 2) * sizeof(float)) != cudaSuccess ||
        cudaMallocHost((void**)&h->pm_cnt[j], 8 * sizeof(long long)) != cudaSuccess)
      return bail(b2g_fail(B2G_ECUDA, "pipelined-path resources"));
  }
  if (cudaStreamCreateWithFlags(&h->cstream, cudaStreamNonBlocking) != cudaSuccess) return bail(b2g_fail(B2G_ECUDA, "copy stream"));
  {
    const char* fk = getenv("B2G_FORK");
    if (!(fk && atoi(fk) == 0)) {
      if (cudaStreamCreateWithFlags(&h->aux, cudaStreamNonBlocking) != cudaSuccess ||
          cudaStreamCreateWithFlags(&h->aux2, cudaStreamNonBlocking) != cudaSuccess) return bail(b2g_fail(B2G_ECUDA, "aux stream"));
      for (auto& e : h->ev_aux)
        if (cudaEventCreateWithFlags(&e, cudaEventDisableTiming) != cudaSuccess) return bail(b2g_fail(B2G_ECUDA, "aux events"));
      h->fork_leaves = true;
    }
  }
  {
    std::vector<double> ones(h->Ec, 1.0);
    if (cudaMemcpyAsync(h->d_istd, ones.data(), h->Ec * sizeof(double), cudaMemcpyHostToDevice, h->stream) != cudaSuccess ||
        cudaStreamSynchronize(h->stream) != cudaSuccess)
      return bail(b2g_fail(B2G_ECUDA, "init copy failed"));
  }
  if ((rc = build_groups(h))) return bail(rc);
  if (h->v2.on && (rc = v2_create(h))) return bail(rc);
  if (cfg->nranks > 1) {
    if (!cfg->nccl_id) return bail(b2g_fail(B2G_EINVAL, "nranks > 1 needs nccl_id"));
    if ((rc = nccl_comm_init(&h->nccl_comm, cfg->nranks, cfg->nccl_id, cfg->rank, cfg->nccl_lib))) return bail(rc);
    {
      const char* ov = getenv("B2G_AR_OVERLAP");
      const bool want_ov = h->v2.on && !(ov && ov[0] == '0');
      if (want_ov && g_nccl.CommSplit && g_nccl.GroupStart && g_nccl.GroupEnd) {
        if (g_nccl.CommSplit(h->nccl_comm, 0, cfg->rank, &h->nccl_comm2, nullptr) == 0 && h->nccl_comm2 &&
            cudaStreamCreateWithFlags(&h->side, cudaStreamNonBlocking) == cudaSuccess &&
            cudaEventCreateWithFlags(&h->ev_fork, cudaEventDisableTiming) == cudaSuccess &&
            cudaEventCreateWithFlags(&h->ev_join, cudaEventDisableTiming) == cudaSuccess) {
          h->overlap_ar = true;
          if (const char* e = getenv("B2G_AR_SMS")) h->ar_sms = atoi(e);
          g_nccl.AllReduce(h->G, h->G, 1024, 7, 0, h->nccl_comm2, h->side);
          cudaStreamSynchronize(h->side);
        }
      }
    }
    const int nrc = g_nccl.AllReduce(h->G, h->G, (size_t)(h->n_train + MET_COUNT), 7, 0, h->nccl_comm, h->stream);
    if (nrc != 0 || cudaStreamSynchronize(h->stream) != cudaSuccess) return bail(b2g_fail(B2G_ENCCL, "NCCL warm-up all-reduce failed"));
  }
  const char* ng = getenv("B2G_NO_GRAPH");
  h->use_graph = !(ng && ng[0] == '1');
  if (cudaStreamSynchronize(h->stream) != cudaSuccess) return bail(b2g_fail(B2G_ECUDA, "create: sync failed"));
  *out = h;
  return 0;
}

int b2g_sync(b2g_sac* h) {
  B2G_USABLE(h);
  if (!h) return b2g_fail(B2G_EINVAL, "NULL handle");
  CK(cudaSetDevice(h->cfg.device));
  CK(cudaStreamSynchronize(h->stream));
  return 0;
}

int b2g_param_count(const b2g_sac* h) { B2G_USABLE(h); return h ? (int)h->tensors.size() : 0; }

int b2g_param_info(const b2g_sac* h, int idx, const char** name, int64_t* numel, int32_t* ndim, int64_t shape[4]) {
  B2G_USABLE(h);
  if (!h || idx < 0 || idx >= (int)h->tensors.size()) return b2g_fail(B2G_EINVAL, "bad tensor index");
  const Tensor& t = h->tensors[idx];
  if (name) *name = t.name.c_str();
  if (numel) *numel = t.numel;
  if (ndim) *ndim = t.ndim;
  if (shape) for (int i = 0; i < 4; ++i) shape[i] = t.shape[i];
  return 0;
}

static int copy_tensor(b2g_sac* h, const char* name, float* arena, float* host, size_t numel, bool to_host, bool trainable_only) {
  if (!h || !host) return b2g_fail(B2G_EINVAL, "NULL argument");
  const int i = find_tensor(h, name);
  if (i < 0) return b2g_fail(B2G_EINVAL, std::string("unknown variable: ") + (name ? name : "(null)"));
  const Tensor& t = h->tensors[i];
  if ((int64_t)numel != t.numel) return b2g_fail(B2G_EINVAL, std::string("size mismatch for ") + t.name);
  if (trainable_only && t.group == 3) return b2g_fail(B2G_EINVAL, std::string("not a trainable variable: ") + t.name);
  CK(cudaSetDevice(h->cfg.device));
  CK(cudaStreamSynchronize(h->stream));
  if (to_host) CK(cudaMemcpy(host, arena + t.off, numel * sizeof(float), cudaMemcpyDeviceToHost));
  else CK(cudaMemcpy(arena + t.off, host, numel * sizeof(float), cudaMemcpyHostToDevice));
  return 0;
}

int b2g_get_param(b2g_sac* h, const char* name, float* dst, size_t numel) { B2G_USABLE(h); return copy_tensor(h, name, h ? h->P : nullptr, dst, numel, true, false); }
int b2g_set_param(b2g_sac* h, const char* name, const float* src, size_t numel) {
  B2G_USABLE(h);
  int rc = copy_tensor(h, name, h ? h->P : nullptr, const_cast<float*>(src), numel, false, false);
  if (rc == 0) h->planes_dirty = true;
  return rc;
}
int b2g_get_grad(b2g_sac* h, const char* name, float* dst, size_t numel) {
  B2G_USABLE(h);
  int rc = copy_tensor(h, name, h ? h->G : nullptr, dst, numel, true, true);
  if (rc == 0 && h->cfg.nranks > 1) for (size_t i = 0; i < numel; ++i) dst[i] /= (float)h->cfg.nranks;
  return rc;
}
int b2g_get_adam(b2g_sac* h, const char* name, float* m, float* v, size_t numel) {
  B2G_USABLE(h);
  if (int rc = copy_tensor(h, name, h ? h->Mo : nullptr, m, numel, true, true)) return rc;
  return copy_tensor(h, name, h->Vo, v, numel, true, true);
}
int b2g_reset_optimizer(b2g_sac* h) {
  B2G_USABLE(h);
  if (!h) return b2g_fail(B2G_EINVAL, "NULL handle");
  CK(cudaSetDevice(h->cfg.device));
  CK(cudaMemsetAsync(h->Mo, 0, h->n_train * sizeof(float), h->stream));
  CK(cudaMemsetAsync(h->Vo, 0, h->n_train * sizeof(float), h->stream));
  CK(cudaMemsetAsync(h->counters, 0, 4 * sizeof(long long), h->stream));
  CK(cudaStreamSynchronize(h->stream));
  return 0;
}

int b2g_replay_add(b2g_sac* h, const float* obs, const float* act, const float* rew, const float* next_obs, const float* done,
                   int64_t n) {
  B2G_USABLE(h);
  if (!h || !obs || !act || !rew || !next_obs || !done || n < 0) return b2g_fail(B2G_EINVAL, "NULL argument");
  if (h->dedup && 2 * n > h->frame_cap) return b2g_fail(B2G_EINVAL, "replay_add: 2 n rows exceed frame_capacity");
  CK(cudaSetDevice(h->cfg.device));
  const int64_t FC = h->frame_cap;
  const int64_t R = commit_rows(h);
  const size_t E = h->E, A = h->A;
  const FrameIo io = frame_io(h, h->c_obs, h->c_next);
  int* flags = h->h_plan + 3 * R;
  auto stage_check = [&](int64_t c0, int m, bool check) -> int {
    if (c0 > 0) CK(cudaStreamSynchronize(h->stream));
    if (int rc = load_rows(h, obs + c0 * E, h->c_obs, 0, R, m)) return rc;
    if (int rc = load_rows(h, next_obs + c0 * E, h->c_next, 0, R, m)) return rc;
    if (!check) return 0;
    for (int i = 0; i < m; ++i) {
      const int64_t p = c0 + i < (int64_t)h->prev_next.size() ? h->prev_next[c0 + i] : -1;
      h->h_plan[i] = h->dedup && p >= 0 && p > h->next_fid - FC ? (int)(p % FC) : -1;
    }
    CK(cudaMemcpyAsync(h->d_plan, h->h_plan, m * sizeof(int), cudaMemcpyHostToDevice, h->stream));
    frame_check_launch(io, h->d_plan, h->d_plan + 3 * R, m, h->stream);
    CK(cudaMemcpyAsync(flags, h->d_plan + 3 * R, m * sizeof(int), cudaMemcpyDeviceToHost, h->stream));
    CK(cudaStreamSynchronize(h->stream));
    for (int i = 0; i < m; ++i)
      if (flags[i] & 2) return b2g_fail(B2G_EINVAL, "replay_add: a value of an 8-bit plane is not an integer in [0, 255]");
    return 0;
  };
  if (h->u8_mask && n > R)
    for (int64_t c0 = 0; c0 < n; c0 += R)
      if (int rc = stage_check(c0, (int)std::min<int64_t>(R, n - c0), true)) return rc;
  std::vector<int64_t> next_ids((size_t)n), cand((size_t)R);
  for (int64_t c0 = 0; c0 < n; c0 += R) {
    const int m = (int)std::min<int64_t>(R, n - c0);
    if (int rc = stage_check(c0, m, h->dedup || (h->u8_mask && n <= R))) return rc;
    for (int i = 0; i < m; ++i) {
      const int64_t p = c0 + i < (int64_t)h->prev_next.size() ? h->prev_next[c0 + i] : -1;
      cand[i] = h->dedup && (flags[i] & 1) ? p : -1;
    }
    if (int rc = commit_chunk(h, io, m, cand.data(), act + c0 * A, rew + c0, done + c0, next_ids.data() + c0)) return rc;
  }
  h->up_other += (int64_t)(n * (2 * E + A + 2) * sizeof(float));
  if (int rc = commit_finish(h, next_ids)) return rc;
  CK(cudaStreamSynchronize(h->stream));
  return 0;
}

int64_t b2g_replay_size(const b2g_sac* h) { B2G_USABLE(h); return h ? h->r_size : 0; }

int b2g_replay_info(const b2g_sac* h, int64_t* capacity, int64_t* size, int64_t* frame_capacity, int64_t* live_frames,
                    int64_t* bytes, int64_t* evicted_early) {
  B2G_USABLE(h);
  if (!h) return b2g_fail(B2G_EINVAL, "NULL handle");
  const int64_t cap = h->cfg.buffer_capacity;
  int64_t live = 0;
  if (h->r_size > 0) {
    int64_t lo = h->next_fid;
    for (const auto& q : h->lw) if (q.first >= h->tail_seq) { lo = q.second; break; }
    live = h->next_fid - lo;
  }
  if (capacity) *capacity = cap;
  if (size) *size = h->r_size;
  if (frame_capacity) *frame_capacity = h->frame_cap;
  if (live_frames) *live_frames = live;
  if (bytes) *bytes = h->frame_cap * h->frame_bytes + cap * (int64_t)(2 * sizeof(int) + (h->A + 2) * sizeof(float));
  if (evicted_early) *evicted_early = h->evicted;
  return 0;
}

int b2g_replay_get(b2g_sac* h, int64_t slot, float* obs, float* act, float* rew, float* next_obs, float* done) {
  B2G_USABLE(h);
  if (!h) return b2g_fail(B2G_EINVAL, "NULL handle");
  const int64_t cap = h->cfg.buffer_capacity;
  if (slot < 0 || slot >= cap || ((slot - h->tail_seq % cap) % cap + cap) % cap >= h->r_size)
    return b2g_fail(B2G_EINVAL, "replay slot is not live");
  CK(cudaSetDevice(h->cfg.device));
  CK(cudaStreamSynchronize(h->stream));
  const size_t A = h->A;
  std::vector<unsigned char> fr(h->frame_bytes);
  const FrameFmt& fm = h->fmt;
  const int npx = h->cnn ? h->Hi * h->Wi * h->Cimg : 0;
  for (int w = 0; w < 2; ++w) {
// ... 488 lines not shown
```

deep-rl-grasping_b200/csrc/sac_internal.cuh:

```cuda
#pragma once
#include <cuda_runtime.h>

#include <deque>
#include <map>
#include <string>
#include <tuple>
#include <vector>

#include "../../include/b200grasp.h"
#include "cg.cuh"
#include "common.cuh"
#include "host.cuh"

namespace b2g {
struct Tensor {
  std::string name;
  int ndim;
  int64_t shape[4];
  int64_t numel;
  int64_t off;
  int group;
};


__host__ __device__ constexpr int s2d_channels(int Ci) { return Ci == 1 ? 1 : 4; }
__host__ __device__ inline int conv1_krow(int r, int Ci) {
  const int ci = r % Ci, kx = (r / Ci) % 8, ky = r / (8 * Ci);
  return ((((ky >> 2) * 2 + (kx >> 2)) * 4 + (ky & 3)) * 4 + (kx & 3)) * s2d_channels(Ci) + ci;
}
struct V2State {
  bool on = false;
  int KF = 576;
  uint16_t* S[2][3]{};
  uint16_t* H1[3][3]{};
  uint16_t* H2[3][3]{};
  uint16_t* H3[3][3]{};
  uint16_t* F[3][3]{};
  uint16_t* dz0pi[2]{};
  uint16_t* dz0v[2]{};
  uint16_t* dZ4[2][2]{};
  uint16_t* dZ3[2][2]{};
  uint16_t* dZ2[2][2]{};
  uint16_t* dZ1[2]{};
  uint16_t* W1T[2][3]{};
  uint16_t* W2T[3][3]{};
  uint16_t* W3T[3][3]{};
  uint16_t* WfT[3][3]{};
  uint16_t* K0T[3][3]{};
  uint16_t* W2n[2][2]{};
  uint16_t* W3n[2][2]{};
  uint16_t* Wfn[2][2]{};
  uint16_t* K0n[2][2]{};
  float* z0v = nullptr;
  void* plane_jobs = nullptr; int n_plane_jobs = 0, plane_ctas = 0;
  int plane_ctas_fwd = 0;
  const int* plane_cta_job = nullptr;
  int sm_reserve = 0;
  std::vector<CUtensorMap> maps;
  std::vector<char> map_whole;
  std::vector<int> map_box_bytes;
  CUtensorMap* d_maps = nullptr;
  std::vector<CgGroup> fwd, bwd_groups;
  std::vector<CgGroup> fwd_fused, bwd_fused;
  int split_fc1 = 3;
  int split_fc1_dgrad = 1;
  int* dep_ctr = nullptr; int n_dep_ctr = 0;
  std::vector<int*> tabs;
  int dbg = 0;
};

}

struct b2g_sac;
namespace b2g {
int v2_alloc(b2g_sac* h);
int v2_create(b2g_sac* h);
int v2_planes(b2g_sac* h, bool backward, cudaStream_t s);
int v2_gather(b2g_sac* h, const GatherArgs& ga, cudaStream_t s);
int v2_launch(b2g_sac* h, const CgGroup& g, cudaStream_t s);
int sac_act_rows(b2g_sac* h, const float* rows, int chunk, int deterministic);
int sac_replay_add_linked(b2g_sac* h, const float* c_obs, const float* c_next, const int64_t* obs_fid, const float* act,
                          const float* rew, const float* done, int n, int64_t* next_fid);
void obs_rms_derive(b2g_sac* h);
}

using namespace b2g;

struct b2g_sac {
  b2g_sac_cfg cfg{};
  bool cnn = false;
  int num_sms = 132;
  int B = 0, A = 0, H = 0, E = 0, Cimg = 0, feat_dim = 0, FS = 0;
  int Hi = 0, Wi = 0, H1 = 0, W1 = 0, H2 = 0, W2 = 0, H3 = 0, W3 = 0;
  std::vector<Tensor> tensors;
  std::map<std::string, int> tindex;
  int64_t n_pi = 0, n_values = 0, n_ent = 0, n_target = 0, n_train = 0, n_all = 0;
  float *P = nullptr, *Mo = nullptr, *Vo = nullptr, *G = nullptr;
  float* metrics = nullptr;
  cudaStream_t stream = nullptr;
  std::vector<void*> allocs;
  int Ec = 0;
  unsigned char* frames = nullptr;
  int64_t frame_cap = 0, frame_bytes = 0;
  FrameFmt fmt{}, row_fmt{};
  uint32_t u8_mask = 0;
  bool dedup = false;
  int *r_ofr = nullptr, *r_nfr = nullptr;
  float *r_act = nullptr, *r_rew = nullptr, *r_done = nullptr;
  int64_t r_size = 0, head_seq = 0, tail_seq = 0, next_fid = 0, evicted = 0;
  std::deque<std::pair<int64_t, int64_t>> lw;
  std::vector<int64_t> prev_next;
  float *c_obs = nullptr, *c_next = nullptr;
  int *d_plan = nullptr, *h_plan = nullptr;
  long long* h_rc = nullptr;
  float* obs_stage = nullptr;
  int stage_rows = 0;
  double *d_mean = nullptr, *d_istd = nullptr, *d_normc = nullptr;
  double ret_istd = 1.0, clip_obs = 10.0, clip_rew = 10.0;
  int norm_obs = 0, norm_rew = 0;
  float *x_obs = nullptr, *x_next = nullptr;
  float *h1[3]{}, *h2[3]{}, *h3[3]{}, *F[3]{};
  float *dZ4[2]{}, *dZ3p[2]{}, *dZ2p[2]{}, *dZ1[2]{};
  float *z0[5]{}, *a0[4]{}, *dz1[4]{}, *dz0_pi = nullptr, *dz0_v3 = nullptr;
  bool use_planes = false;
  uint16_t *xp[2][2]{}, *h1p[3][2]{}, *h2p[3][2]{}, *h3p[3][2]{};
  uint16_t *dZ4p[2][2]{}, *dZ3pp[2][2]{}, *dZ2pp[2][2]{}, *dZ1p[2][2]{};
  ColsumJob* d_colsum = nullptr;
  int n_colsum = 0, colsum_ctas = 0;
  uint16_t* wp[3][4][4]{};
  PlaneJob* d_jobs = nullptr;
  int n_jobs = 0, job_tiles = 0;
  bool planes_dirty = true;
  std::map<const int*, std::vector<int>> host_tabs;
  float *per_sample = nullptr, *pi_out = nullptr, *eps = nullptr, *rew_n = nullptr, *done_n = nullptr;
  int* indices = nullptr;
  float *s_obs = nullptr, *s_next = nullptr, *s_act = nullptr, *s_rew = nullptr, *s_done = nullptr;
  float *ps_obs[2]{}, *ps_next[2]{};
  float *hc_obs[2]{}, *hc_next[2]{};
  cudaGraphExec_t pipe_graph[2]{};
  int host_threads = 16;
  cudaStream_t cstream = nullptr;
  cudaEvent_t ev_h2d[2]{}, ev_consumed[2]{}, ev_met[2]{};
  float* pm_met[2]{};
  long long* pm_cnt[2]{};
  long long pipe_k = 0;
  bool pipe_pending = false;
  cudaEvent_t record_after_gather = nullptr;
  long long* counters = nullptr;
  double* step_consts = nullptr;
  float* d_lr = nullptr;
  float cur_lr = -1.f;
  std::vector<GemmGroup> fwd_groups, bwd_groups, act_groups;
  cudaGraphExec_t graph_exec = nullptr;
  bool use_graph = true;
  void* nccl_comm = nullptr;
  void* nccl_comm2 = nullptr;
  bool pipe_serial = false; int pipe_tune = 0; double pipe_t0 = 0, pipe_period[2] = {0, 0};
  bool dp_p2p = false;
  int* dp_x = nullptr;
  int* dp_sync = nullptr;
  float* dp_recv = nullptr;
  float* dp_P[8]{}; float* dp_G[8]{}; int* dp_X[8]{};
  std::vector<void*> dp_opened;
  int dp_skip[2][2]{};
  cudaStream_t side = nullptr;
  cudaStream_t aux = nullptr;
  cudaStream_t aux2 = nullptr;
  cudaEvent_t ev_aux[9]{};
  bool fork_leaves = false;
  std::map<std::tuple<const void*, const void*, const void*, int>, int> col_ids;
  cudaEvent_t ev_fork = nullptr, ev_join = nullptr;
  bool overlap_ar = false;
  int ar_sms = 8;
  ColsumJob* d_colsum_early = nullptr;
  int n_colsum_early = 0, colsum_early_ctas = 0;
  cudaEvent_t ev0 = nullptr, ev1 = nullptr;
  float last_ms = 0.f;
  int launches = 0;
  std::vector<std::string> prof_names;
  float* h_met = nullptr;
  long long* h_cnt = nullptr;

  b2g::V2State v2;
  bool broken = false;
  double* hp_stats[2]{};
  cudaEvent_t ev_stats[2]{};
  int stats_k = 0;
  double norm_eps = 1e-8;

  double *rms_mean = nullptr, *rms_var = nullptr;
  double rms_count = 0.0;
  float* ob_full[2]{};
  float* ob_rows[2]{};
  int ob_k = 0;
  float *ob_act = nullptr, *ob_rew = nullptr, *ob_done = nullptr;
  std::vector<int64_t> ob_fid;
  int ob_n = 0;
  int64_t up_observe = 0, up_other = 0;

  float* p(const std::string& n) { return P + tensors[tindex.at(n)].off; }
  float* g(const std::string& n) { return G + tensors[tindex.at(n)].off; }
};
```

include/b200grasp.h:

```cpp
#ifndef B200GRASP_H_
#define B200GRASP_H_

#include <stddef.h>
#include <stdint.h>

#ifdef __cplusplus
extern "C" {
#endif

#define B2G_OK 0
#define B2G_EINVAL (-1)
#define B2G_ECUDA (-2)
#define B2G_ESTATE (-3)
#define B2G_ENCCL (-4)

#define B2G_PREC_FP32_SIMT 0
#define B2G_PREC_BF16X3 1
#define B2G_PREC_BF16 2

typedef struct b2g_sac b2g_sac;

typedef struct b2g_sac_cfg {
  int32_t obs_h, obs_w, obs_c;
  int32_t obs_dim;
  int32_t n_act;
  int32_t hidden;
  int32_t batch;
  int64_t buffer_capacity;
  float gamma, tau, target_entropy;
  uint64_t seed;
  int32_t precision;
  int32_t device;
  int32_t rank, nranks;
  const void* nccl_id;
  const char* nccl_lib;
} b2g_sac_cfg;

typedef struct b2g_sac_metrics {
  float policy_loss, qf1_loss, qf2_loss, value_loss, ent_coef_loss, entropy, ent_coef;
  float grad_norm_pi, grad_norm_values, grad_ent;
  float mean_q1, mean_q2, mean_v, mean_logp;
  int64_t n_updates;
} b2g_sac_metrics;

const char* b2g_last_error(void);
int b2g_version(void);
int b2g_nccl_unique_id(void* out128, const char* nccl_lib);

typedef struct b2g_replay_cfg {
  int64_t frame_capacity;
  uint32_t u8_plane_mask;
} b2g_replay_cfg;

int b2g_sac_create(const b2g_sac_cfg* cfg, b2g_sac** out);
int b2g_sac_create2(const b2g_sac_cfg* cfg, const b2g_replay_cfg* replay , b2g_sac** out);
int b2g_sac_destroy(b2g_sac* h);
#define B2G_DP_EXPORT_BYTES 192
int b2g_sac_dp_export(b2g_sac* h, void* out192);
int b2g_sac_dp_connect(b2g_sac* h, const void* all_exports , int nranks);
int b2g_debug_dp_stamps(b2g_sac* h, long long* out5);
int b2g_debug_compact_host(const float* src, float* dst, int n, int hw, int cfull, int threads);
int b2g_sync(b2g_sac* h);

int b2g_param_count(const b2g_sac* h);
int b2g_param_info(const b2g_sac* h, int idx, const char** name, int64_t* numel, int32_t* ndim, int64_t shape[4]);
int b2g_get_param(b2g_sac* h, const char* name, float* dst, size_t numel);
int b2g_set_param(b2g_sac* h, const char* name, const float* src, size_t numel);
int b2g_get_grad(b2g_sac* h, const char* name, float* dst, size_t numel);
int b2g_get_adam(b2g_sac* h, const char* name, float* m, float* v, size_t numel);
int b2g_reset_optimizer(b2g_sac* h);

int b2g_replay_add(b2g_sac* h, const float* obs, const float* act, const float* rew, const float* next_obs,
                   const float* done, int64_t n);
int64_t b2g_replay_size(const b2g_sac* h);
int b2g_replay_get(b2g_sac* h, int64_t slot, float* obs, float* act, float* rew, float* next_obs, float* done);
int b2g_replay_info(const b2g_sac* h, int64_t* capacity, int64_t* size, int64_t* frame_capacity, int64_t* live_frames,
                    int64_t* bytes, int64_t* evicted_early);
int b2g_get_last_batch(b2g_sac* h, int32_t* indices, float* eps, float* per_sample, float* pi_out);
int b2g_set_norm_stats(b2g_sac* h, const double* obs_mean, const double* obs_var, double ret_var, double clip_obs,
                       double clip_rew, double eps, int norm_obs, int norm_reward);

int b2g_sac_observe_act(b2g_sac* h, const float* obs, int n, int update_stats, int deterministic, float* act_out);
int b2g_sac_observe_add(b2g_sac* h, const float* act, const float* rew, const float* next_obs, const float* done,
                        const float* reset_obs , int n, int update_stats);
int b2g_obs_rms_set(b2g_sac* h, const double* mean, const double* var, double count);
int b2g_obs_rms_get(b2g_sac* h, double* mean, double* var, double* count);
int b2g_upload_bytes(const b2g_sac* h, int64_t* observe_bytes, int64_t* other_bytes);

int b2g_sac_step(b2g_sac* h, int n_steps, float lr, b2g_sac_metrics* out);
int b2g_sac_step_async(b2g_sac* h, int n_steps, float lr);

int b2g_sac_step_explicit(b2g_sac* h, const float* obs, const float* act, const float* rew, const float* next_obs,
                          const float* done, const float* eps, float lr, int apply_update, b2g_sac_metrics* out,
                          float* per_sample, float* pi_out);

int b2g_sac_step_host_pipelined(b2g_sac* h, const float* obs, const float* act, const float* rew, const float* next_obs,
                                const float* done, const float* eps, float lr, b2g_sac_metrics* prev_out, int* have_prev);
int b2g_sac_pipeline_flush(b2g_sac* h, b2g_sac_metrics* last_out);

int b2g_sac_act(b2g_sac* h, const float* obs, int n, int deterministic, float* act_out);

int b2g_sac_state_save(b2g_sac* h, const char* path);
int b2g_sac_state_load(b2g_sac* h, const char* path);

int b2g_launches_per_step(const b2g_sac* h);
float b2g_last_step_ms(const b2g_sac* h);
int b2g_profile_step(b2g_sac* h, float lr, const char** names, float* ms, int cap);

typedef struct b2g_bdq b2g_bdq;
typedef struct b2g_bdq_cfg {
  int32_t obs_dim;
  int32_t n_branches;
  int32_t n_bins;
  int32_t trunk0, trunk1;
  int32_t branch_hidden;
  int32_t batch;
  int64_t buffer_capacity;
  float gamma;
  int32_t target_update_freq;
  int32_t trunk_grad_rescale;
  uint64_t seed;
  int32_t device;
  int32_t rank, nranks;
  const void* nccl_id;
  const char* nccl_lib;
  int32_t prioritized_replay;
  float per_alpha, per_eps;
} b2g_bdq_cfg;
typedef struct b2g_bdq_metrics {
  float loss, mean_q, grad_norm;
  int64_t n_updates;
} b2g_bdq_metrics;

int b2g_bdq_create(const b2g_bdq_cfg* cfg, b2g_bdq** out);
int b2g_bdq_destroy(b2g_bdq* h);
int b2g_bdq_param_count(const b2g_bdq* h);
int b2g_bdq_param_info(const b2g_bdq* h, int idx, char* name, size_t name_cap, int64_t* rows, int64_t* cols, int32_t* ndim);
int b2g_bdq_get_param(b2g_bdq* h, const char* name, float* dst, size_t numel);
int b2g_bdq_set_param(b2g_bdq* h, const char* name, const float* src, size_t numel);
int b2g_bdq_get_grad(b2g_bdq* h, const char* name, float* dst, size_t numel);
int b2g_bdq_replay_add(b2g_bdq* h, const float* obs, const float* act_idx, const float* rew, const float* next_obs,
                       const float* done, int64_t n);
int64_t b2g_bdq_replay_size(const b2g_bdq* h);
int b2g_bdq_set_norm_stats(b2g_bdq* h, const double* obs_mean, const double* obs_var, double ret_var, double clip_obs,
                           double clip_rew, double eps, int norm_obs, int norm_reward);
int b2g_bdq_step(b2g_bdq* h, int n_steps, float lr, b2g_bdq_metrics* out);
int b2g_bdq_set_per_beta(b2g_bdq* h, float beta);
int b2g_bdq_get_last_per(b2g_bdq* h, int32_t* slots, float* weights, float* priorities);
int b2g_bdq_step_explicit(b2g_bdq* h, const float* obs, const float* act_idx, const float* rew, const float* next_obs,
                          const float* done, const float* weights, float lr, int apply_update, b2g_bdq_metrics* out,
                          float* td_out);
int b2g_bdq_act(b2g_bdq* h, const float* obs, int n, int32_t* act_idx_out);

int b2g_bdq_observe_act(b2g_bdq* h, const float* obs, int n, int update_stats, float eps, int32_t* act_idx_out);
int b2g_bdq_observe_add(b2g_bdq* h, const float* act_idx, const float* rew, const float* next_obs, const float* done,
                        const float* reset_obs , int n, int update_stats);
int b2g_bdq_obs_rms_set(b2g_bdq* h, const double* mean, const double* var, double count);
int b2g_bdq_obs_rms_get(b2g_bdq* h, double* mean, double* var, double* count);
int b2g_bdq_upload_bytes(const b2g_bdq* h, int64_t* observe_bytes, int64_t* other_bytes);
int b2g_bdq_state_save(b2g_bdq* h, const char* path);
int b2g_bdq_state_load(b2g_bdq* h, const char* path);

typedef struct b2g_dqn b2g_dqn;
typedef struct b2g_dqn_cfg {
  int32_t obs_dim;
  int32_t n_actions;
  int32_t hidden0, hidden1;
  int32_t batch;
  int64_t buffer_capacity;
  float gamma;
  uint64_t seed;
  int32_t device;
  int32_t prioritized_replay;
  float per_alpha, per_eps;
} b2g_dqn_cfg;
typedef struct b2g_dqn_metrics {
  float loss;
  float mean_q, mean_abs_td;
  float grad_norm;
  int32_t n_clipped;
  int64_t n_updates;
} b2g_dqn_metrics;

int b2g_dqn_create(const b2g_dqn_cfg* cfg, b2g_dqn** out);
int b2g_dqn_destroy(b2g_dqn* h);
int b2g_dqn_param_count(const b2g_dqn* h);
int b2g_dqn_param_info(const b2g_dqn* h, int idx, char* name, size_t name_cap, int64_t* rows, int64_t* cols, int32_t* ndim);
int b2g_dqn_get_param(b2g_dqn* h, const char* name, float* dst, size_t numel);
int b2g_dqn_set_param(b2g_dqn* h, const char* name, const float* src, size_t numel);
int b2g_dqn_get_grad(b2g_dqn* h, const char* name, float* dst, size_t numel);
int b2g_dqn_replay_add(b2g_dqn* h, const float* obs, const float* act, const float* rew, const float* next_obs, const float* done,
                       int64_t n);
int64_t b2g_dqn_replay_size(const b2g_dqn* h);
int b2g_dqn_set_norm_stats(b2g_dqn* h, const double* obs_mean, const double* obs_var, double ret_var, double clip_obs,
                           double clip_rew, double eps, int norm_obs, int norm_reward);
int b2g_dqn_step(b2g_dqn* h, int n_steps, float lr, b2g_dqn_metrics* out);
int b2g_dqn_set_per_beta(b2g_dqn* h, float beta);
int b2g_dqn_get_last_per(b2g_dqn* h, int32_t* slots, float* weights, float* priorities);
int b2g_dqn_step_explicit(b2g_dqn* h, const float* obs, const float* act, const float* rew, const float* next_obs, const float* done,
                          const float* weights, float lr, int apply_update, b2g_dqn_metrics* out, float* td_out);
int b2g_dqn_update_target(b2g_dqn* h);
int b2g_dqn_act(b2g_dqn* h, const float* obs, int n, int32_t* act_out, float* q_out);
int b2g_dqn_state_save(b2g_dqn* h, const char* path);
int b2g_dqn_state_load(b2g_dqn* h, const char* path);

typedef struct b2g_ppo b2g_ppo;
typedef struct b2g_ppo_cfg {
  int32_t obs_dim;
  int32_t n_actions;
  int32_t hidden0, hidden1;
  int32_t n_envs;
  int32_t n_steps;
  int32_t nminibatches;
  int32_t noptepochs;
  float gamma, lam;
  float ent_coef, vf_coef;
  float max_grad_norm;
  uint64_t seed;
  int32_t device;
} b2g_ppo_cfg;
typedef struct b2g_ppo_metrics {
  float policy_loss, value_loss, entropy, approxkl, clipfrac;
  float grad_norm;
  int64_t n_updates;
} b2g_ppo_metrics;

int b2g_ppo_create(const b2g_ppo_cfg* cfg, b2g_ppo** out);
int b2g_ppo_destroy(b2g_ppo* h);
int b2g_ppo_param_count(const b2g_ppo* h);
int b2g_ppo_param_info(const b2g_ppo* h, int idx, char* name, size_t name_cap, int64_t* rows, int64_t* cols, int32_t* ndim);
int b2g_ppo_get_param(b2g_ppo* h, const char* name, float* dst, size_t numel);
int b2g_ppo_set_param(b2g_ppo* h, const char* name, const float* src, size_t numel);
int b2g_ppo_get_grad(b2g_ppo* h, const char* name, float* dst, size_t numel);
int b2g_ppo_rollout_act(b2g_ppo* h, const float* obs, float* act_out);
int b2g_ppo_rollout_reward(b2g_ppo* h, const float* rew, const float* done);
int b2g_ppo_rollout_reset(b2g_ppo* h);
int b2g_ppo_rollout_get(b2g_ppo* h, float* adv, float* ret, float* val, float* nlp, float* act);
int b2g_ppo_update(b2g_ppo* h, const float* last_obs, const int32_t* perm, float lr, float cliprange, float cliprange_vf,
                   b2g_ppo_metrics* out);
int b2g_ppo_train_step_explicit(b2g_ppo* h, const float* obs, const float* returns, const float* actions, const float* values,
                                const float* neglogp, float lr, float cliprange, float cliprange_vf, int apply_update,
                                b2g_ppo_metrics* out);
int b2g_ppo_act(b2g_ppo* h, const float* obs, int n, int deterministic, float* act_out, float* value_out, float* neglogp_out);
int b2g_ppo_get_step(b2g_ppo* h, int64_t* adam_step, int64_t* noise_step, int32_t* rollout_rows);
int b2g_ppo_state_save(b2g_ppo* h, const char* path);
int b2g_ppo_state_load(b2g_ppo* h, const char* path);

#define B2G_ENC_MAX_LAYERS 8
typedef struct b2g_encoder b2g_encoder;
typedef struct b2g_encoder_cfg {
  int32_t height, width, channels;
  int32_t n_layers;
  int32_t filters[B2G_ENC_MAX_LAYERS];
  int32_t kernel[B2G_ENC_MAX_LAYERS];
  int32_t strides[B2G_ENC_MAX_LAYERS];
  int32_t encoding_dim;
  float alpha;
  int32_t max_batch;
  int32_t device;
} b2g_encoder_cfg;
// ... 35 lines not shown
```

Baseline: 2568.

## Replace round-robin tile striding with host-built cost-model tile schedule per CTA

Each CTA of the persistent grouped GEMM kernel now walks a precomputed list of tiles instead of striding by gridDim. The host builds these lists once at creation from a cost model that accounts for fill, repartition, chunk cycles and inter-problem dependencies, then uploads them. The aim is to balance load across CTAs and order tiles so dependency waits and smem repartitions are reduced. It also adds per-tile tracing kernels and debug APIs, and the Walker can now jump to arbitrary problems. The cost is extra device table reads and a schedule that may be poorly tuned for H100.

```diff
diff --git a/deep-rl-grasping_b200/_lib.py b/deep-rl-grasping_b200/_lib.py
--- a/deep-rl-grasping_b200/_lib.py
+++ b/deep-rl-grasping_b200/_lib.py
@@ -29,6 +29,7 @@
     "b2g_ppo_update", "b2g_ppo_train_step_explicit", "b2g_ppo_act", "b2g_ppo_get_step", "b2g_ppo_state_save", "b2g_ppo_state_load",
     "b2g_encoder_create", "b2g_encoder_destroy", "b2g_encoder_n_layers", "b2g_encoder_layer_shape", "b2g_encoder_set_weights",
     "b2g_encoder_encode", "b2g_debug_gemm", "b2g_debug_tensor_info", "b2g_debug_tensor",
+    "b2g_cg_schedule", "b2g_cg_schedule_check", "b2g_debug_cg_schedule", "b2g_debug_cg_tiles",
     "b2g_autoencoder_create", "b2g_autoencoder_destroy", "b2g_autoencoder_n_layers", "b2g_autoencoder_layer_shape",
     "b2g_autoencoder_set_weights", "b2g_autoencoder_get_weights", "b2g_autoencoder_get_grad", "b2g_autoencoder_reset_optimizer",
     "b2g_autoencoder_set_dataset", "b2g_autoencoder_train_epoch", "b2g_autoencoder_evaluate", "b2g_autoencoder_predict",
@@ -250,6 +251,11 @@
     lib.b2g_debug_gemm.argtypes = [C.c_int, C.c_int, C.c_int, fp, fp, fp, C.c_int, C.c_int]
     lib.b2g_debug_tensor_info.argtypes = [vp, C.c_char_p, i64p, C.POINTER(C.c_int32), C.POINTER(C.c_int32)]
     lib.b2g_debug_tensor.argtypes = [vp, C.c_char_p, C.c_int, vp, C.c_size_t]
+    ip = C.POINTER(C.c_int)
+    lib.b2g_cg_schedule.argtypes = [ip, C.c_int, C.c_int, ip, ip, ip, C.c_int]
+    lib.b2g_cg_schedule_check.argtypes = [ip, C.c_int, C.c_int, ip, ip, ip, C.c_int]
+    lib.b2g_debug_cg_schedule.argtypes = [vp, C.c_char_p, ip, ip, C.c_int]
+    lib.b2g_debug_cg_tiles.argtypes = [vp, C.c_char_p, C.POINTER(C.c_longlong), C.c_int]
     _lib = lib
     return lib
 
diff --git a/deep-rl-grasping_b200/csrc/cg.cu b/deep-rl-grasping_b200/csrc/cg.cu
--- a/deep-rl-grasping_b200/csrc/cg.cu
+++ b/deep-rl-grasping_b200/csrc/cg.cu
@@ -82,16 +82,15 @@
 struct Walker {
   int p = -1, next_start = 0, tile_start = 0, tiles_n = 1, per = 1, splits = 1, chunks = 0, cps = 0;
   __device__ __forceinline__ bool advance(const CgProblem* __restrict__ probs, int nprob, int tile) {
-    bool changed = false;
-    while (p < 0 || (p + 1 < nprob && tile >= next_start)) {
-      ++p;
-      const CgProblem& P = probs[p];
-      tile_start = P.tile_start; tiles_n = P.tiles_n; per = P.tiles_m * P.tiles_n; splits = P.splits; chunks = P.chunks;
-      cps = (chunks + splits - 1) / splits;
-      next_start = p + 1 < nprob ? probs[p + 1].tile_start : 0x7fffffff;
-      changed = true;
-    }
-    return changed;
+    if (p >= 0 && tile >= tile_start && tile < next_start) return false;
+    int q = 0;
+    while (q + 1 < nprob && tile >= probs[q + 1].tile_start) ++q;
+    p = q;
+    const CgProblem& P = probs[p];
+    tile_start = P.tile_start; tiles_n = P.tiles_n; per = P.tiles_m * P.tiles_n; splits = P.splits; chunks = P.chunks;
+    cps = (chunks + splits - 1) / splits;
+    next_start = p + 1 < nprob ? probs[p + 1].tile_start : 0x7fffffff;
+    return true;
   }
   __device__ __forceinline__ Tile tile(int t_abs) const {
     int t = t_abs - tile_start, split = 0;
@@ -147,6 +146,11 @@
       "}" ::"r"(bar), "r"((uint32_t)pred)
       : "memory");
 }
+__device__ __forceinline__ long long gtimer() {
+  long long t;
+  asm volatile("mov.u64 %0, %%globaltimer;" : "=l"(t));
+  return t;
+}
 __device__ __forceinline__ void stamp_if(long long* dst, bool pred) {
   asm volatile(
       "{\n\t"
@@ -162,7 +166,8 @@
 template <int NT, int NPROD, int TRANS, int KS, class Body>
 __device__ __forceinline__ void consume_tile(const CgProblem& P, const Tile& ti, uint32_t ring, uint32_t stg, int slot_bytes, int nstages, uint32_t& s,
                                              uint32_t& ph, uint64_t* bar_full, uint64_t* bar_empty, bool nomma, long long* ctrace, uint32_t& gc,
-                                             bool handoff, uint32_t acc_buf, uint32_t& nb, uint64_t* acc_full, uint64_t* acc_empty, Body&& body) {
+                                             bool handoff, uint32_t acc_buf, uint32_t& nb, uint64_t* acc_full, uint64_t* acc_empty, Body&& body,
+                                             long long* trec) {
   constexpr int NGRP = NPROD >= 6 ? 3 : (NPROD >= 3 ? 2 : 1);
   constexpr int NACC = NT / 2 * NGRP;
   const int tid = threadIdx.x, lane = tid & 31, warp = tid >> 5;
@@ -202,6 +207,7 @@
     wg_wait<0>();
     mbar_arrive_if(smem_u32(&bar_empty[prev]), lane == 0);
   }
+  if (trec && tid == 0) { trec[CG_TR_MMA_LAST] = gtimer(); trec[CG_TR_MMA_CLK1] = clock64(); }
   if constexpr (NGRP > 2) {
 #pragma unroll
     for (int j = 0; j < NT / 2; ++j) acc[j] = acc[j] + (acc[j + NT / 2] + acc[j + NT]);
@@ -275,17 +281,21 @@
   }
 };
 
-__global__ void __launch_bounds__(NTHREADS, 1)
-cg_kernel(const __grid_constant__ CgPack pk, int nprob, int total_tiles, const CUtensorMap* __restrict__ maps, int max_stages,
-          int dbg, long long* __restrict__ trace) {
+template <bool TRACE>
+__device__ __forceinline__ void cg_body(const CgPack& pk, int nprob, const int* __restrict__ sched, const int* __restrict__ cta_begin,
+                                        const CUtensorMap* __restrict__ maps, int max_stages, int dbg, long long* __restrict__ trace,
+                                        long long* __restrict__ ttrace_arg) {
   const CgProblem* __restrict__ probs = pk.p;
+  long long* __restrict__ const ttrace = TRACE ? ttrace_arg : nullptr;
   extern __shared__ uint8_t smem_raw[];
   __shared__ __align__(8) uint64_t bar_full[CG_MAX_STAGES], bar_empty[CG_MAX_STAGES], acc_full, acc_empty;
+  __shared__ int list_end;
   const int tid = threadIdx.x, lane = tid & 31;
   const int warp = __shfl_sync(0xffffffffu, tid >> 5, 0);
   const int trace_cta = dbg >> 8;
   const bool dbg_noload = dbg & 1, dbg_nomma = dbg & 2, dbg_nostore = dbg & 4, dbg_nost = dbg & 16;
   if (tid == 0) {
+    list_end = cta_begin[blockIdx.x + 1];
     for (int s = 0; s < max_stages; ++s) { mbar_init(smem_u32(&bar_full[s]), 1); mbar_init(smem_u32(&bar_empty[s]), NMMA_WARPS); }
     mbar_init(smem_u32(&acc_full), NMMA_WARPS);
     mbar_init(smem_u32(&acc_empty), NEPI_WARPS);
@@ -296,6 +306,7 @@
   const uint32_t ring = stg + STG_BYTES;
   pdl_trigger();
   pdl_wait();
+  const int k0 = cta_begin[blockIdx.x];
 
   if (warp >= PROD_WARP0) {
     asm volatile("setmaxnreg.dec.sync.aligned.u32 %0;" ::"n"(PROD_REGS));
@@ -308,11 +319,16 @@
       Walker w;
       int n2 = 1, nloads = 0, planes = 0, tx = 0;
       const int* tab = nullptr;
-      for (int tile = blockIdx.x; tile < total_tiles; tile += gridDim.x) {
+      int next = sched[k0];
+      for (int k = k0; k < *(volatile int*)&list_end; ++k) {
+        const int tile = next;
+        next = sched[k + 1];
+        bool repart = false;
         if (w.advance(probs, nprob, tile)) {
           const CgProblem& P = probs[w.p];
           n2 = P.n2; nloads = P.nloads; planes = P.planes; tx = P.tx_bytes; tab = P.tm_tab; handoff = cg_epi_handoff(P.epi);
           if (P.slot_bytes != slot_bytes || P.nstages != nstages) {
+            repart = slot_bytes != 0;
             for (int q = 0; q < nstages; ++q) mbar_wait(smem_u32(&bar_empty[q]), ((ph >> q) & 1u) ^ 1u);
             if (nbuf) {
               mbar_wait(smem_u32(&acc_full), (nbuf - 1) & 1u);
@@ -325,6 +341,11 @@
         const Tile ti = w.tile(tile);
         const CgProblem& P = probs[ti.p];
         if (handoff && ti.c_end > ti.c_begin) ++nbuf;
+        long long* const trec = ttrace && pw == 0 && lane == 0 ? ttrace + (size_t)tile * CG_TILE_REC : nullptr;
+        if (trec) {
+          trec[CG_TR_CTA] = blockIdx.x; trec[CG_TR_PROB] = ti.p; trec[CG_TR_REPART] = repart; trec[CG_TR_CHUNKS] = ti.c_end - ti.c_begin;
+          trec[CG_TR_DEP_WAIT] = gtimer();
+        }
         if (P.dep_ctr) {
           const int* __restrict__ ctr = P.dep_ctr;
           const int x0 = P.dep_by_chunk ? ti.c_begin : ti.tm, x1 = P.dep_by_chunk ? ti.c_end : ti.tm + 1;
@@ -340,6 +361,7 @@
           __syncwarp();
           asm volatile("fence.proxy.async.global;" ::: "memory");
         }
+        if (trec) trec[CG_TR_DEP_DONE] = gtimer();
         int base[CG_MAX_LOADS][5];
 #pragma unroll
         for (int l = 0; l < CG_MAX_LOADS; ++l) {
@@ -404,7 +426,10 @@
     uint32_t acc_buf = 0;
     long long o_tm = 0;
     RowOff ro;
-    for (int tile = blockIdx.x; tile < total_tiles; tile += gridDim.x) {
+    int next = sched[k0];
+    for (int k = k0; k < *(volatile int*)&list_end; ++k) {
+      const int tile = next;
+      next = sched[k + 1];
       if (w.advance(probs, nprob, tile)) {
         const CgProblem& Q = probs[w.p];
         epi = Q.epi; rows_tile = Q.rows_tile; lim_rows = Q.lim_rows; umma_n = Q.umma_n; n_valid = Q.n_valid; o_tm = Q.o_tm;
@@ -422,6 +447,11 @@
       const int n0 = ti.tn * umma_n;
       const bool tre = trace && blockIdx.x == trace_cta && warp == 0 && lane == 0 && it < 16;
       if (tre) trace[512 + it * 4 + 0] = clock64();
+      long long* const trec = ttrace ? ttrace + (size_t)tile * CG_TILE_REC : nullptr;
+      if (trec && !dbg_nomma) {
+        mbar_wait(smem_u32(&bar_full[s]), (ph >> s) & 1u);
+        if (tid == 0) { trec[CG_TR_MMA_FIRST] = gtimer(); trec[CG_TR_MMA_CLK0] = clock64(); }
+      }
       auto body = [&](int g, float (&x)[32]) {
         const int ng = n0 + 32 * g;
         if (dbg_nostore || ng >= n_valid || !valid0) return;
@@ -464,7 +494,7 @@
       };
 #define CG_CONSUME(NT, NPROD, TRANS, KS)                                                                                                      \
   consume_tile<NT, NPROD, TRANS, KS>(P, ti, ring, stg, slot_bytes, nstages, s, ph, bar_full, bar_empty, dbg_nomma, ctrace, gc, handoff, acc_buf, \
-                                     nb, &acc_full, &acc_empty, body)
+                                     nb, &acc_full, &acc_empty, body, trec)
       switch (shape) {
         case cg_shape_key(32, 6, false, 4): CG_CONSUME(32, 6, 0, 4); break;
         case cg_shape_key(64, 6, false, 4): CG_CONSUME(64, 6, 0, 4); break;
@@ -476,6 +506,10 @@
         default: __trap();
       }
 #undef CG_CONSUME
+      if (trec && !handoff && tid == 0) {
+        trec[CG_TR_EPI_START] = trec[CG_TR_MMA_LAST]; trec[CG_TR_EPI_CLK0] = trec[CG_TR_MMA_CLK1];
+        trec[CG_TR_EPI_END] = gtimer(); trec[CG_TR_EPI_CLK1] = clock64();
+      }
       if (tre) {
         trace[512 + it * 4 + 1] = clock64();
         trace[512 + it * 4 + 2] = handoff;
@@ -497,7 +531,10 @@
     RowOff ro;
     const float* __restrict__ bias = nullptr;
     const uint16_t* __restrict__ mask = nullptr;
-    for (int tile = blockIdx.x; tile < total_tiles; tile += gridDim.x) {
+    int next = sched[k0];
+    for (int k = k0; k < *(volatile int*)&list_end; ++k) {
+      const int tile = next;
+      next = sched[k + 1];
       if (w.advance(probs, nprob, tile)) {
         const CgProblem& Q = probs[w.p];
         epi = Q.epi; rows_tile = Q.rows_tile; lim_rows = Q.lim_rows; umma_n = Q.umma_n; out_planes = Q.out_planes;
@@ -556,6 +593,10 @@
       }
       mbar_wait(smem_u32(&acc_full), ne & 1u);
       if (tre) trace[576 + ne * 4 + 1] = clock64();
+      if (ttrace && ew == 0 && lane == 0) {
+        long long* const trec = ttrace + (size_t)tile * CG_TILE_REC;
+        trec[CG_TR_EPI_START] = gtimer(); trec[CG_TR_EPI_CLK0] = clock64();
+      }
       const bool split_fin = P.ws != nullptr;
       float* __restrict__ wsrow = split_fin ? P.ws + ((size_t)(ti.tm * w.tiles_n + ti.tn) * 128 + r) * umma_n : nullptr;
       auto body = [&](int g, float (&x)[32], int pass) {
@@ -688,9 +729,24 @@
         __threadfence();
         atomicAdd(P.done_ctr + ti.tm, 1);
       }
+      if (ttrace && ew == 0 && lane == 0) {
+        long long* const trec = ttrace + (size_t)tile * CG_TILE_REC;
+        trec[CG_TR_EPI_END] = gtimer(); trec[CG_TR_EPI_CLK1] = clock64();
+      }
       if (tre) { trace[576 + (ne - 1) * 4 + 2] = clock64(); trace[576 + (ne - 1) * 4 + 3] = ti.p * 100000 + ti.tm * 10 + ti.tn; }
     }
   }
+}
+
+__global__ void __launch_bounds__(NTHREADS, 1)
+cg_kernel(const __grid_constant__ CgPack pk, int nprob, const int* __restrict__ sched, const int* __restrict__ cta_begin,
+          const CUtensorMap* __restrict__ maps, int max_stages, int dbg, long long* __restrict__ trace) {
+  cg_body<false>(pk, nprob, sched, cta_begin, maps, max_stages, dbg, trace, nullptr);
+}
+__global__ void __launch_bounds__(NTHREADS, 1)
+cg_tile_trace_kernel(const __grid_constant__ CgPack pk, int nprob, const int* __restrict__ sched, const int* __restrict__ cta_begin,
+                     const CUtensorMap* __restrict__ maps, int max_stages, int dbg, long long* __restrict__ trace, long long* __restrict__ ttrace) {
+  cg_body<true>(pk, nprob, sched, cta_begin, maps, max_stages, dbg, trace, ttrace);
 }
 
 typedef CUresult (*EncodeTiledFn)(CUtensorMap*, CUtensorMapDataType, cuuint32_t, void*, const cuuint64_t*, const cuuint64_t*, const cuuint32_t*,
@@ -770,20 +826,29 @@
 
 long long* g_cg_trace = nullptr;
 
-cudaError_t cg_launch(const CgGroup& g, const CUtensorMap* dev_maps, int num_sms, cudaStream_t s, bool pdl, int debug_flags) {
+cudaError_t cg_launch(const CgGroup& g, const CUtensorMap* dev_maps, int num_sms, cudaStream_t s, bool pdl, int debug_flags,
+                      long long* tile_trace) {
   if (g.total_tiles <= 0 || (debug_flags & 8)) return cudaSuccess;
+  if (!g.sched || !g.cta_begin || g.ctas != (g.total_tiles < num_sms ? g.total_tiles : num_sms)) {
+    fprintf(stderr, "cg_launch %s: no tile schedule for %d SMs (built for %d CTAs)\n", g.name, num_sms, g.ctas);
+    return cudaErrorInvalidConfiguration;
+  }
   static bool attr_set = false;
   if (!attr_set) {
     cudaError_t e = cudaFuncSetAttribute(cg_kernel, cudaFuncAttributeMaxDynamicSharedMemorySize, 226 * 1024);
+    if (e == cudaSuccess) e = cudaFuncSetAttribute(cg_tile_trace_kernel, cudaFuncAttributeMaxDynamicSharedMemorySize, 226 * 1024);
     if (e != cudaSuccess) return e;
     attr_set = true;
   }
   const int smem = 1024 + STG_BYTES + g.ring_bytes;
-  const int grid = g.total_tiles < num_sms ? g.total_tiles : num_sms;
+  const int grid = g.ctas;
   CgPack pk;
   static_assert(sizeof(CgPack) < 28 * 1024, "problem list must fit the kernel parameter space (32,764 B)");
   for (int i = 0; i < g.n; ++i) pk.p[i] = g.host[i];
-  cudaError_t e = launch_pdl(cg_kernel, dim3(grid), dim3(NTHREADS), (size_t)smem, s, pdl, pk, g.n, g.total_tiles, dev_maps, g.nstages, debug_flags, g_cg_trace);
+  cudaError_t e = tile_trace ? launch_pdl(cg_tile_trace_kernel, dim3(grid), dim3(NTHREADS), (size_t)smem, s, pdl, pk, g.n, g.sched, g.cta_begin,
+                                          dev_maps, g.nstages, debug_flags, g_cg_trace, tile_trace)
+                             : launch_pdl(cg_kernel, dim3(grid), dim3(NTHREADS), (size_t)smem, s, pdl, pk, g.n, g.sched, g.cta_begin, dev_maps,
+                                          g.nstages, debug_flags, g_cg_trace);
   if (e != cudaSuccess) fprintf(stderr, "cg_launch %s: %s (grid %d, %d threads, smem %d)\n", g.name, cudaGetErrorString(e), grid, NTHREADS, smem);
   return e;
 }
diff --git a/deep-rl-grasping_b200/csrc/cg.cuh b/deep-rl-grasping_b200/csrc/cg.cuh
--- a/deep-rl-grasping_b200/csrc/cg.cuh
+++ b/deep-rl-grasping_b200/csrc/cg.cuh
@@ -2,6 +2,8 @@
 #include <cuda.h>
 #include <cuda_runtime.h>
 #include <stdint.h>
+
+#include <vector>
 
 namespace b2g {
 
@@ -96,13 +98,29 @@
   int slot_bytes = 0, nstages = 0, ring_bytes = 0;
   const char* name = "";
   double flops = 0;
+  const int* sched = nullptr;
+  const int* cta_begin = nullptr;
+  int ctas = 0;
+  std::vector<int> h_sched, h_cta_begin;
+};
+enum CgTileRec : int {
+  CG_TR_CTA = 0, CG_TR_PROB,
+  CG_TR_DEP_WAIT, CG_TR_DEP_DONE,
+  CG_TR_REPART,
+  CG_TR_MMA_FIRST, CG_TR_MMA_LAST,
+  CG_TR_MMA_CLK0, CG_TR_MMA_CLK1,
+  CG_TR_EPI_START, CG_TR_EPI_END,
+  CG_TR_EPI_CLK0, CG_TR_EPI_CLK1,
+  CG_TR_CHUNKS,
+  CG_TILE_REC = 16
 };
 
 int cg_encode_map(CUtensorMap* out, const void* base, int rank, const uint64_t* dims, const uint64_t* strides_bytes, const uint32_t* box,
                   const uint32_t* elem_strides, int swizzle = 128);
 unsigned long long cg_desc_bits(int swizzle, bool mn_major, int lbo);
 int cg_finalize(CgGroup& g, int smem_budget);
-cudaError_t cg_launch(const CgGroup& g, const CUtensorMap* dev_maps, int num_sms, cudaStream_t s, bool pdl, int debug_flags);
+cudaError_t cg_launch(const CgGroup& g, const CUtensorMap* dev_maps, int num_sms, cudaStream_t s, bool pdl, int debug_flags,
+                      long long* tile_trace = nullptr);
 int cg_smem_limit();
 __host__ __device__ constexpr int cg_shape_key(int umma_n, int nprod, bool mn_major, int ksteps) {
   return ksteps * 8192 + umma_n * 16 + nprod * 2 + (mn_major ? 1 : 0);
diff --git a/deep-rl-grasping_b200/csrc/cg_sched.cu b/deep-rl-grasping_b200/csrc/cg_sched.cu
--- /dev/null
+++ b/deep-rl-grasping_b200/csrc/cg_sched.cu
@@ -0,0 +1,273 @@
+#include <algorithm>
+#include <cstdio>
+#include <queue>
+#include <string>
+#include <vector>
+
+#include "cg_sched.cuh"
+
+namespace b2g {
+namespace {
+
+constexpr double FILL = 800.0;
+constexpr double REPARTITION = 2000.0;
+constexpr double TMA_BYTES_PER_CYCLE = 23.0;
+double chunk_cycles(const SchedProblem& p) { return std::max(600.0 + 1.9 * p.ksteps * p.nprod * p.umma_n, p.tx_bytes / TMA_BYTES_PER_CYCLE); }
+double epi_cycles(const SchedProblem& p) {
+  if (!p.handoff) return 1000.0 + 100.0 * p.umma_n;
+  return 2000.0 + 40.0 * p.umma_n * p.out_planes + (p.out_planes == 2 ? 60.0 * p.umma_n : 0.0);
+}
+
+struct TileRef { int p, tm, c_begin, c_end; };
+TileRef decode(const SchedProblem& P, int t) {
+  const int per = P.tiles_m * P.tiles_n, cps = (P.chunks + P.splits - 1) / P.splits;
+  const int split = t / per, r = t - split * per;
+  TileRef x;
+  x.p = -1; x.tm = r / P.tiles_n;
+  x.c_begin = split * cps; x.c_end = std::min(P.chunks, x.c_begin + cps);
+  return x;
+}
+
+struct Dag {
+  std::vector<int> start, prob;
+  std::vector<int> pred_begin, pred;
+  int total = 0;
+};
+
+int build_dag(const std::vector<SchedProblem>& probs, Dag& d, std::string& err) {
+  const int n = (int)probs.size();
+  d.start.assign(n + 1, 0);
+  for (int i = 0; i < n; ++i) {
+    const SchedProblem& P = probs[i];
+    if (P.tiles_m < 1 || P.tiles_n < 1 || P.splits < 1 || P.chunks < 0) { err = "problem " + std::to_string(i) + " has an empty tile grid"; return -1; }
+    d.start[i + 1] = d.start[i] + P.tiles_m * P.tiles_n * P.splits;
+  }
+  d.total = d.start[n];
+  d.prob.resize(d.total);
+  for (int i = 0; i < n; ++i) std::fill(d.prob.begin() + d.start[i], d.prob.begin() + d.start[i + 1], i);
+  std::vector<std::vector<int>> signallers(n);
+  for (int c = 0; c < n; ++c) {
+    if (probs[c].dep_id < 0) continue;
+    for (int q = 0; q < n; ++q)
+      if (probs[q].done_id == probs[c].dep_id) {
+        if (q >= c) {
+          err = "problem " + std::to_string(c) + " waits on problem " + std::to_string(q) + ", which is not listed before it";
+          return -1;
+        }
+        if (!probs[q].handoff) { err = "problem " + std::to_string(q) + " is wired as a producer but its epilogue signals no counter"; return -1; }
+        if (probs[q].tiles_m != probs[c].dep_tiles) { err = "problem " + std::to_string(c) + " counts its producer's row tiles wrong"; return -1; }
+        signallers[c].push_back(q);
+      }
+    if (signallers[c].empty()) { err = "problem " + std::to_string(c) + " waits on counters no problem of the launch signals"; return -1; }
+  }
+  d.pred_begin.assign(d.total + 1, 0);
+  d.pred.clear();
+  for (int t = 0; t < d.total; ++t) {
+    const int c = d.prob[t];
+    const SchedProblem& P = probs[c];
+    if (P.dep_id >= 0) {
+      const TileRef x = decode(P, t - d.start[c]);
+      const int x0 = P.dep_by_chunk ? x.c_begin : x.tm, x1 = P.dep_by_chunk ? x.c_end : x.tm + 1;
+      const int lo = x0 * P.dep_rows / P.dep_rows_tile, hi = std::min(P.dep_tiles - 1, (x1 * P.dep_rows - 1) / P.dep_rows_tile);
+      for (int q : signallers[c]) {
+        const SchedProblem& Q = probs[q];
+        const int per = Q.tiles_m * Q.tiles_n;
+        for (int j = lo; j <= hi; ++j)
+          for (int s = 0; s < Q.splits; ++s)
+            for (int tn = 0; tn < Q.tiles_n; ++tn) d.pred.push_back(d.start[q] + s * per + j * Q.tiles_n + tn);
+      }
+    }
+    d.pred_begin[t + 1] = (int)d.pred.size();
+  }
+  return 0;
+}
+
+}
+
+int cg_schedule_check(const std::vector<SchedProblem>& probs, int num_ctas, const CgSchedule& s, std::string& err) {
+  Dag d;
+  if (build_dag(probs, d, err)) return -1;
+  const int T = d.total;
+  if ((int)s.order.size() != T || (int)s.sched.size() != T || (int)s.cta_begin.size() != num_ctas + 1 || s.cta_begin[0] != 0 ||
+      s.cta_begin[num_ctas] != T) {
+    err = "schedule sizes do not match the launch's " + std::to_string(T) + " tiles on " + std::to_string(num_ctas) + " CTAs";
+    return -1;
+  }
+  std::vector<int> rank(T, -1);
+  for (int k = 0; k < T; ++k) {
+    const int t = s.order[k];
+    if (t < 0 || t >= T) { err = "tile id " + std::to_string(t) + " out of range"; return -1; }
+    if (rank[t] >= 0) { err = "tile " + std::to_string(t) + " appears twice in the global order"; return -1; }
+    rank[t] = k;
+  }
+  std::vector<char> seen(T, 0);
+  for (int c = 0; c < num_ctas; ++c) {
+    if (s.cta_begin[c + 1] < s.cta_begin[c]) { err = "CTA list bounds decrease"; return -1; }
+    for (int k = s.cta_begin[c]; k < s.cta_begin[c + 1]; ++k) {
+      const int t = s.sched[k];
+      if (t < 0 || t >= T) { err = "tile id " + std::to_string(t) + " out of range"; return -1; }
+      if (seen[t]) { err = "tile " + std::to_string(t) + " is dealt twice"; return -1; }
+      seen[t] = 1;
+      if (k > s.cta_begin[c] && rank[s.sched[k - 1]] >= rank[t]) {
+        err = "the list of CTA " + std::to_string(c) + " is not increasing in the global order at tile " + std::to_string(t);
+        return -1;
+      }
+    }
+  }
+  for (int t = 0; t < T; ++t) {
+    if (!seen[t]) { err = "tile " + std::to_string(t) + " is missing from the CTA lists"; return -1; }
+    for (int e = d.pred_begin[t]; e < d.pred_begin[t + 1]; ++e)
+      if (rank[d.pred[e]] >= rank[t]) {
+        err = "tile " + std::to_string(t) + " waits on tile " + std::to_string(d.pred[e]) + ", which is not earlier in the global order";
+        return -1;
+      }
+  }
+  return 0;
+}
+
+int cg_schedule_build(const std::vector<SchedProblem>& probs, int num_ctas, CgSchedule& out, std::string& err) {
+  if (num_ctas < 1) { err = "a schedule needs at least one CTA"; return -1; }
+  Dag d;
+  if (build_dag(probs, d, err)) return -1;
+  const int T = d.total;
+  std::vector<int> succ_begin(T + 1, 0), succ(d.pred.size()), npred(T, 0);
+  for (int t = 0; t < T; ++t)
+    for (int e = d.pred_begin[t]; e < d.pred_begin[t + 1]; ++e) ++succ_begin[d.pred[e] + 1];
+  for (int t = 0; t < T; ++t) succ_begin[t + 1] += succ_begin[t];
+  {
+    std::vector<int> fill(succ_begin.begin(), succ_begin.end() - 1);
+    for (int t = 0; t < T; ++t)
+      for (int e = d.pred_begin[t]; e < d.pred_begin[t + 1]; ++e) succ[fill[d.pred[e]]++] = t;
+  }
+  std::vector<double> busy(T), tail(T), blevel(T);
+  for (int t = 0; t < T; ++t) {
+    const SchedProblem& P = probs[d.prob[t]];
+    const TileRef x = decode(P, t - d.start[d.prob[t]]);
+    const int nch = std::max(0, x.c_end - x.c_begin);
+    npred[t] = d.pred_begin[t + 1] - d.pred_begin[t];
+    if (nch == 0) { busy[t] = tail[t] = 0.0; continue; }
+    busy[t] = FILL + nch * chunk_cycles(P) + (P.handoff ? 0.0 : epi_cycles(P));
+    tail[t] = P.handoff ? epi_cycles(P) : 0.0;
+  }
+  for (int t = T - 1; t >= 0; --t) {
+    double m = 0.0;
+    for (int e = succ_begin[t]; e < succ_begin[t + 1]; ++e) m = std::max(m, blevel[succ[e]]);
+    blevel[t] = busy[t] + tail[t] + m;
+  }
+  std::vector<double> ready_at(T, 0.0), cta_free(num_ctas, 0.0), epi_free(num_ctas, 0.0);
+  std::vector<int> cta_part(num_ctas, -1), cta_of(T, -1);
+  auto by_ready = [&](int a, int b) { return ready_at[a] > ready_at[b] || (ready_at[a] == ready_at[b] && a > b); };
+  auto by_level = [&](int a, int b) { return blevel[a] < blevel[b] || (blevel[a] == blevel[b] && a > b); };
+  std::priority_queue<int, std::vector<int>, decltype(by_ready)> pending(by_ready);
+  std::priority_queue<int, std::vector<int>, decltype(by_level)> ready(by_level);
+  for (int t = 0; t < T; ++t)
+    if (npred[t] == 0) pending.push(t);
+  out.order.clear();
+  out.order.reserve(T);
+  while ((int)out.order.size() < T) {
+    int c = 0;
+    for (int k = 1; k < num_ctas; ++k)
+      if (cta_free[k] < cta_free[c]) c = k;
+    double now = cta_free[c];
+    while (!pending.empty() && ready_at[pending.top()] <= now) { ready.push(pending.top()); pending.pop(); }
+    if (ready.empty()) {
+      if (pending.empty()) { err = "the tile dependencies form a cycle"; return -1; }
+      now = ready_at[pending.top()];
+      while (!pending.empty() && ready_at[pending.top()] <= now) { ready.push(pending.top()); pending.pop(); }
+    }
+    const int t = ready.top();
+    ready.pop();
+    const SchedProblem& P = probs[d.prob[t]];
+    const int part = P.slot_bytes * 16 + P.nstages;
+    const double start = std::max(now, ready_at[t]) + (cta_part[c] >= 0 && cta_part[c] != part ? REPARTITION : 0.0);
+    cta_part[c] = part;
+    double done = start + busy[t];
+    cta_free[c] = done;
+    if (tail[t] > 0.0) {
+      const double epi_start = std::max(done, epi_free[c]);
+      cta_free[c] = epi_start;
+      done = epi_free[c] = epi_start + tail[t];
+    }
+    cta_of[t] = c;
+    out.order.push_back(t);
+    for (int e = succ_begin[t]; e < succ_begin[t + 1]; ++e) {
+      const int s = succ[e];
+      ready_at[s] = std::max(ready_at[s], done);
+      if (--npred[s] == 0) pending.push(s);
+    }
+  }
+  out.makespan = std::max(*std::max_element(cta_free.begin(), cta_free.end()), *std::max_element(epi_free.begin(), epi_free.end()));
+  out.cta_begin.assign(num_ctas + 1, 0);
+  for (int t = 0; t < T; ++t) ++out.cta_begin[cta_of[t] + 1];
+  for (int c = 0; c < num_ctas; ++c) out.cta_begin[c + 1] += out.cta_begin[c];
+  out.sched.assign(T, 0);
+  std::vector<int> fill(out.cta_begin.begin(), out.cta_begin.end() - 1);
+  for (int t : out.order) out.sched[fill[cta_of[t]]++] = t;
+  return cg_schedule_check(probs, num_ctas, out, err);
+}
+
+std::vector<SchedProblem> cg_sched_problems(const CgGroup& g) {
+  std::vector<const int*> ids;
+  auto id_of = [&](const int* p) -> int {
+    if (!p) return -1;
+    for (size_t i = 0; i < ids.size(); ++i) if (ids[i] == p) return (int)i;
+    ids.push_back(p);
+    return (int)ids.size() - 1;
+  };
+  std::vector<SchedProblem> out(g.n);
+  for (int i = 0; i < g.n; ++i) {
+    const CgProblem& P = g.host[i];
+    SchedProblem& s = out[i];
+    s.tiles_m = P.tiles_m; s.tiles_n = P.tiles_n; s.splits = P.splits; s.chunks = P.chunks;
+    s.handoff = cg_epi_handoff(P.epi) ? 1 : 0; s.umma_n = P.umma_n; s.nprod = P.nprod; s.ksteps = P.ksteps;
+    s.tx_bytes = P.tx_bytes; s.slot_bytes = P.slot_bytes; s.nstages = P.nstages; s.out_planes = P.out_planes;
+    s.done_id = id_of(P.done_ctr); s.dep_id = id_of(P.dep_ctr);
+    s.dep_rows = P.dep_rows; s.dep_rows_tile = P.dep_rows_tile; s.dep_tiles = P.dep_tiles; s.dep_by_chunk = P.dep_by_chunk;
+  }
+  return out;
+}
+
+}
+
+namespace b2g {
+std::vector<SchedProblem> sched_table(const int* geom, int nprob) {
+  std::vector<SchedProblem> probs(nprob);
+  for (int i = 0; i < nprob; ++i) {
+    const int* r = geom + i * B2G_SCHED_FIELDS;
+    SchedProblem& s = probs[i];
+    s.tiles_m = r[0]; s.tiles_n = r[1]; s.splits = r[2]; s.chunks = r[3]; s.handoff = r[4]; s.umma_n = r[5]; s.nprod = r[6];
+    s.ksteps = r[7]; s.tx_bytes = r[8]; s.slot_bytes = r[9]; s.nstages = r[10]; s.out_planes = r[11]; s.done_id = r[12];
+    s.dep_id = r[13]; s.dep_rows = r[14]; s.dep_rows_tile = r[15]; s.dep_tiles = r[16]; s.dep_by_chunk = r[17];
+  }
+  return probs;
+}
+}
+
+extern "C" int b2g_cg_schedule(const int* geom, int nprob, int num_ctas, int* order, int* sched, int* cta_begin, int cap) {
+  using namespace b2g;
+  if (!geom || nprob < 1 || nprob > CG_MAX_PROBLEMS) return b2g_fail(B2G_EINVAL, "b2g_cg_schedule: 1 .. 16 problems");
+  const std::vector<SchedProblem> probs = b2g::sched_table(geom, nprob);
+  CgSchedule s;
+  std::string err;
+  if (cg_schedule_build(probs, num_ctas, s, err)) return b2g_fail(B2G_EINVAL, "b2g_cg_schedule: " + err);
+  const int T = (int)s.order.size();
+  if (T > cap) return b2g_fail(B2G_EINVAL, "b2g_cg_schedule: " + std::to_string(T) + " tiles exceed the output capacity");
+  if (order) std::copy(s.order.begin(), s.order.end(), order);
+  if (sched) std::copy(s.sched.begin(), s.sched.end(), sched);
+  if (cta_begin) std::copy(s.cta_begin.begin(), s.cta_begin.end(), cta_begin);
+  return T;
+}
+
+extern "C" int b2g_cg_schedule_check(const int* geom, int nprob, int num_ctas, const int* order, const int* sched, const int* cta_begin, int ntiles) {
+  using namespace b2g;
+  if (!geom || !order || !sched || !cta_begin || nprob < 1 || nprob > CG_MAX_PROBLEMS || num_ctas < 1 || ntiles < 0)
+    return b2g_fail(B2G_EINVAL, "b2g_cg_schedule_check: bad arguments");
+  const std::vector<SchedProblem> probs = b2g::sched_table(geom, nprob);
+  CgSchedule s;
+  s.order.assign(order, order + ntiles);
+  s.sched.assign(sched, sched + ntiles);
+  s.cta_begin.assign(cta_begin, cta_begin + num_ctas + 1);
+  std::string err;
+  if (cg_schedule_check(probs, num_ctas, s, err)) return b2g_fail(B2G_EINVAL, "b2g_cg_schedule_check: " + err);
+  return 0;
+}
diff --git a/deep-rl-grasping_b200/csrc/cg_sched.cuh b/deep-rl-grasping_b200/csrc/cg_sched.cuh
--- /dev/null
+++ b/deep-rl-grasping_b200/csrc/cg_sched.cuh
@@ -0,0 +1,32 @@
+#pragma once
+#include <string>
+#include <vector>
+
+#include "cg.cuh"
+#include "host.cuh"
+
+namespace b2g {
+
+struct SchedProblem {
+  int tiles_m = 1, tiles_n = 1, splits = 1, chunks = 0;
+  int handoff = 0;
+  int umma_n = 64, nprod = 1, ksteps = 4, tx_bytes = 0;
+  int slot_bytes = 0, nstages = 0;
+  int out_planes = 0;
+  int done_id = -1, dep_id = -1;
+  int dep_rows = 0, dep_rows_tile = 1, dep_tiles = 0, dep_by_chunk = 0;
+};
+constexpr int B2G_SCHED_FIELDS = 18;
+
+struct CgSchedule {
+  std::vector<int> order;
+  std::vector<int> sched;
+  std::vector<int> cta_begin;
+  double makespan = 0;
+};
+
+std::vector<SchedProblem> cg_sched_problems(const CgGroup& g);
+int cg_schedule_build(const std::vector<SchedProblem>& probs, int num_ctas, CgSchedule& out, std::string& err);
+int cg_schedule_check(const std::vector<SchedProblem>& probs, int num_ctas, const CgSchedule& s, std::string& err);
+
+}
diff --git a/deep-rl-grasping_b200/csrc/engine_v2.cu b/deep-rl-grasping_b200/csrc/engine_v2.cu
--- a/deep-rl-grasping_b200/csrc/engine_v2.cu
+++ b/deep-rl-grasping_b200/csrc/engine_v2.cu
@@ -5,6 +5,7 @@
 #include <cstdlib>
 #include <cstring>
 
+#include "cg_sched.cuh"
 #include "sac_internal.cuh"
 
 namespace b2g {
@@ -846,6 +847,30 @@
   return 0;
 }
 
+int v2_schedule(b2g_sac* h) {
+  V2State& v = h->v2;
+  auto build = [&](CgGroup& g, int sms) -> int {
+    const int ctas = std::min(g.total_tiles, sms);
+    CgSchedule s;
+    std::string err;
+    if (cg_schedule_build(cg_sched_problems(g), ctas, s, err))
+      return b2g_fail(B2G_EINVAL, std::string("engine v2: tile schedule of ") + g.name + ": " + err);
+    const int *ds = nullptr, *dc = nullptr;
+    std::vector<int> padded(s.sched);
+    padded.push_back(-1);
+    if (int rc = upload_table(h->allocs, h->stream, padded, &ds)) return rc;
+    if (int rc = upload_table(h->allocs, h->stream, s.cta_begin, &dc)) return rc;
+    g.sched = ds; g.cta_begin = dc; g.ctas = ctas;
+    g.h_sched = std::move(s.sched); g.h_cta_begin = std::move(s.cta_begin);
+    return 0;
+  };
+  for (CgGroup& g : v.fwd_fused)
+    if (int rc = build(g, h->num_sms)) return rc;
+  for (size_t i = 0; i < v.bwd_fused.size(); ++i)
+    if (int rc = build(v.bwd_fused[i], h->num_sms - (i == 2 && h->overlap_ar ? h->ar_sms : 0))) return rc;
+  return 0;
+}
+
 int v2_planes(b2g_sac* h, bool backward, cudaStream_t s) {
   V2State& v = h->v2;
   const int cta0 = backward ? v.plane_ctas_fwd : 0, n = backward ? v.plane_ctas - v.plane_ctas_fwd : v.plane_ctas_fwd;
@@ -873,6 +898,8 @@
 
 extern long long* g_cg_trace;
 static long long* s_trace_buf = nullptr;
+static long long* s_tile_buf = nullptr;
+static size_t s_tile_cap = 0;
 
 int v2_launch(b2g_sac* h, const CgGroup& g, cudaStream_t s) {
   const char* tn = getenv("B2G_CG_TRACE");
@@ -882,10 +909,21 @@
     if (!s_trace_buf) cudaMalloc(&s_trace_buf, 640 * sizeof(long long));
     cudaMemsetAsync(s_trace_buf, 0, 640 * sizeof(long long), s);
     g_cg_trace = s_trace_buf;
+    const size_t nrec = (size_t)g.total_tiles * CG_TILE_REC;
+    if (nrec > s_tile_cap) {
+      if (s_tile_buf) cudaFree(s_tile_buf);
+      CK(cudaMalloc(&s_tile_buf, nrec * sizeof(long long)));
+      s_tile_cap = nrec;
+    }
+    CK(cudaMemsetAsync(s_tile_buf, 0, nrec * sizeof(long long), s));
     const char* tc = getenv("B2G_CG_TRACE_CTA");
-    cudaError_t e = cg_launch(g, h->v2.d_maps, h->num_sms - h->v2.sm_reserve, s, false, h->v2.dbg | ((tc ? atoi(tc) : 0) << 8));
+    cudaError_t e = cg_launch(g, h->v2.d_maps, h->num_sms - h->v2.sm_reserve, s, false, h->v2.dbg | ((tc ? atoi(tc) : 0) << 8), s_tile_buf);
     g_cg_trace = nullptr;
     if (e != cudaSuccess) return b2g_fail(B2G_ECUDA, cudaGetErrorString(e));
+    std::vector<long long>& rec = h->v2.tile_trace[g.name];
+    rec.resize(nrec);
+    CK(cudaStreamSynchronize(s));
+    CK(cudaMemcpy(rec.data(), s_tile_buf, nrec * sizeof(long long), cudaMemcpyDeviceToHost));
     static int shots = 0;
     if (shots++ == 3) {
       long long t[640];
@@ -910,3 +948,30 @@
 }
 
 }
+
+extern "C" int b2g_debug_cg_schedule(b2g_sac* h, const char* group, int* sched, int* cta_begin, int cap) {
+  using namespace b2g;
+  if (!h || !group || !h->v2.on) return b2g_fail(B2G_EINVAL, "b2g_debug_cg_schedule: no engine v2 on this handle");
+  for (auto* list : {&h->v2.fwd_fused, &h->v2.bwd_fused})
+    for (const CgGroup& g : *list)
+      if (std::string(g.name) == group) {
+        if ((int)g.h_sched.size() > cap || g.ctas + 1 > cap) return b2g_fail(B2G_EINVAL, "b2g_debug_cg_schedule: capacity too small");
+        if (sched) std::copy(g.h_sched.begin(), g.h_sched.end(), sched);
+        if (cta_begin) std::copy(g.h_cta_begin.begin(), g.h_cta_begin.end(), cta_begin);
+        return g.ctas;
+      }
+  return b2g_fail(B2G_EINVAL, std::string("b2g_debug_cg_schedule: no fused launch ") + group);
+}
+
+extern "C" int b2g_debug_cg_tiles(b2g_sac* h, const char* group, long long* out, int cap) {
+  using namespace b2g;
+  if (!h || !group) return b2g_fail(B2G_EINVAL, "b2g_debug_cg_tiles: NULL argument");
+  auto it = h->v2.tile_trace.find(group);
+  if (it == h->v2.tile_trace.end()) return b2g_fail(B2G_ESTATE, std::string("b2g_debug_cg_tiles: no traced launch of ") + group);
+  const int n = (int)(it->second.size() / CG_TILE_REC);
+  if (out) {
+    if (n > cap) return b2g_fail(B2G_EINVAL, "b2g_debug_cg_tiles: capacity too small");
+    std::copy(it->second.begin(), it->second.end(), out);
+  }
+  return n;
+}
diff --git a/deep-rl-grasping_b200/csrc/sac.cu b/deep-rl-grasping_b200/csrc/sac.cu
--- a/deep-rl-grasping_b200/csrc/sac.cu
+++ b/deep-rl-grasping_b200/csrc/sac.cu
@@ -1295,6 +1295,7 @@
     const int nrc = g_nccl.AllReduce(h->G, h->G, (size_t)(h->n_train + MET_COUNT), 7, 0, h->nccl_comm, h->stream);
     if (nrc != 0 || cudaStreamSynchronize(h->stream) != cudaSuccess) return bail(b2g_fail(B2G_ENCCL, "NCCL warm-up all-reduce failed"));
   }
+  if (h->v2.on && (rc = v2_schedule(h))) return bail(rc);
   const char* ng = getenv("B2G_NO_GRAPH");
   h->use_graph = !(ng && ng[0] == '1');
   if (cudaStreamSynchronize(h->stream) != cudaSuccess) return bail(b2g_fail(B2G_ECUDA, "create: sync failed"));
diff --git a/deep-rl-grasping_b200/csrc/sac_internal.cuh b/deep-rl-grasping_b200/csrc/sac_internal.cuh
--- a/deep-rl-grasping_b200/csrc/sac_internal.cuh
+++ b/deep-rl-grasping_b200/csrc/sac_internal.cuh
@@ -65,6 +65,7 @@
   int split_fc1 = 3;
   int split_fc1_dgrad = 1;
   int* dep_ctr = nullptr; int n_dep_ctr = 0;
+  std::map<std::string, std::vector<long long>> tile_trace;
   std::vector<int*> tabs;
   int dbg = 0;
 };
@@ -75,6 +76,7 @@
 namespace b2g {
 int v2_alloc(b2g_sac* h);
 int v2_create(b2g_sac* h);
+int v2_schedule(b2g_sac* h);
 int v2_planes(b2g_sac* h, bool backward, cudaStream_t s);
 int v2_gather(b2g_sac* h, const GatherArgs& ga, cudaStream_t s);
 int v2_launch(b2g_sac* h, const CgGroup& g, cudaStream_t s);
diff --git a/include/b200grasp.h b/include/b200grasp.h
--- a/include/b200grasp.h
+++ b/include/b200grasp.h
@@ -106,6 +106,11 @@
 int b2g_launches_per_step(const b2g_sac* h);
 float b2g_last_step_ms(const b2g_sac* h);
 int b2g_profile_step(b2g_sac* h, float lr, const char** names, float* ms, int cap);
+
+int b2g_cg_schedule(const int* geom, int nprob, int num_ctas, int* order, int* sched, int* cta_begin, int cap);
+int b2g_cg_schedule_check(const int* geom, int nprob, int num_ctas, const int* order, const int* sched, const int* cta_begin, int ntiles);
+int b2g_debug_cg_schedule(b2g_sac* h, const char* group, int* sched, int* cta_begin, int cap);
+int b2g_debug_cg_tiles(b2g_sac* h, const char* group, long long* out, int cap);
 
 typedef struct b2g_bdq b2g_bdq;
 typedef struct b2g_bdq_cfg {
```

New measurement: 2617, median of 6. 1.02x the previous value.
